# ShigemichiMatsuzaki/MSPL

Hardware: AMD Instinct MI355X
Metric: images/sec pseudo-label gen, ESPDNet-UE s=2.0 480x360(->288x480) bs=16 (higher is better)
Workload: dtype f32; 1 GPU; BASELINE configs[1]: ESPDNet-UE s=2.0 C=13 single-source pseudo-label gen (forward + pred+0.5aux argmax + KL uncertainty + histogram), bs=16/GPU, 16x3x288x480 fp32, hipGraph replay, 3 launches in flight per GPU, 2 consecutive batches of 16 per launch; per_gpu_batch=16, batches_in_flight=3, batches_per_launch=2, classes=13

## Files before the change

### include/mspl_hip.h

```cpp
#ifndef MSPL_HIP_H
#define MSPL_HIP_H

#include <stddef.h>
#include <stdint.h>

#ifdef __cplusplus
extern "C" {
#endif

typedef enum {
    MSPL_OK = 0,
    MSPL_ERR_BAD_SHAPE = -1,
    MSPL_ERR_UNSUPPORTED = -2,
    MSPL_ERR_NULL_POINTER = -3,
    MSPL_ERR_HIP = -4
} mspl_status;

typedef struct {
    const float* scale;
    const float* shift;
    const float* alpha;
    const float* pre_add;
    const float* residual;
    const float* reinf_r;
// ... 46 lines not shown
int mspl_avgpool3x3s2_fwd(const float* x, int32_t N, int32_t C, int32_t H, int32_t W,
                          const mspl_epilogue_t* ep, float* out, void* stream);

int mspl_bilinear_fwd(const float* x, int32_t N, int32_t C, int32_t Hi, int32_t Wi, int32_t Ho,
                      int32_t Wo, int32_t align_corners, const mspl_epilogue_t* ep, float* out, void* stream);

int mspl_decoder_merge_fwd(const float* enc, const float* bu, const float* w3, const float* e_scale, const float* e_shift,
                           const float* e_alpha, const float* gate, const float* b_scale, const float* b_shift,
                           const float* b_alpha, const float* wp, const float* p_scale, const float* p_shift,
                           const float* p_alpha, int32_t N, int32_t Cin, int32_t Cout, int32_t P, int32_t H, int32_t W,
                           float* out, void* stream);

int mspl_adaptive_avgpool_fwd(const float* x, int32_t N, int32_t C, int32_t Hi, int32_t Wi,
                              int32_t Ho, int32_t Wo, const mspl_epilogue_t* ep, float* out,
                              void* stream);

int mspl_pointwise_fwd(const float* x, int32_t N, int32_t C, int32_t HW, const mspl_epilogue_t* ep,
                       float* out, void* stream);

int mspl_gap_gate_fwd(const float* x, const float* w, int32_t N, int32_t Cin, int32_t Cout,
                      int32_t HW, float* mean_ws, float* gate, void* stream);

int mspl_fusion_gate_fwd(const float* z, const float* rgb, const float* depth, int64_t count, float* out, void* stream);
int mspl_fusion_gate_bwd(const float* z, const float* rgb, const float* depth, const float* gy, int64_t count,
                         float* gz, float* grgb, float* gdepth, void* stream);

int mspl_avgpool3x3s2_psum_blocks(int32_t H, int32_t W);
int mspl_avgpool3x3s2_psum_fwd(const float* x, int32_t N, int32_t C, int32_t H, int32_t W, const mspl_epilogue_t* ep, float* out,
                               float* psum, void* stream);
int mspl_gate_from_sums_fwd(const float* psum, const float* w, int32_t N, int32_t Cin, int32_t Cout, int32_t nblk, int32_t HW,
                            float* gate, void* stream);

int mspl_down_head_fits(int32_t N, int32_t nin, int32_t n, int32_t groups, int32_t H, int32_t W, uint32_t launch_flags);
int mspl_down_head_psum_blocks(int32_t H, int32_t W);
int mspl_down_head_fwd(const float* x, const float* wp, const float* pscale, const float* pshift, const float* palpha, int32_t N,
                       int32_t nin, int32_t n, int32_t groups, int32_t H, int32_t W, const mspl_epilogue_t* ep, float* r, float* out,
                       float* psum, void* stream);

int64_t mspl_pyr_down_prep_lds_bytes(int32_t N, int32_t P, int32_t h, int32_t w, int32_t nb, const int32_t* hs,
                                     const int32_t* ws);
int mspl_pyr_down_prep_fwd(const float* x, int32_t N, int32_t P, int32_t h, int32_t w, int32_t nb, const int32_t* hs,
                           const int32_t* ws, const float* const* stage_w, float* const* out, void* stream);
int mspl_pyr_down_prep_train_fwd(const float* x, int32_t N, int32_t P, int32_t h, int32_t w, int32_t nb, const int32_t* hs,
                                 const int32_t* ws, const float* const* stage_w, float* const* out, float* const* pooled,
                                 void* stream);
int mspl_pyr_down_mid_bwd(const float* const* g_e, const float* const* pooled, const float* const* stage_w, int32_t N, int32_t P,
                          int32_t h, int32_t w, int32_t nb, const int32_t* hs, const int32_t* ws, float* const* gw,
                          float* const* gx, void* stream);

int mspl_pyrpool_fused_fwd(const float* x, int32_t N, int32_t P, int32_t h, int32_t w, int32_t nb,
                           const int32_t* hs, const int32_t* ws, const float* const* stage_w,
                           const float* const* down_e, const float* br_scale, const float* br_shift,
                           const float* br_alpha, const float* merge_w, const mspl_epilogue_t* ep,
                           float* out, void* stream);

int mspl_pyrpool_fused_train_fwd(const float* x, int32_t N, int32_t P, int32_t h, int32_t w, int32_t nb,
                                 const int32_t* hs, const int32_t* ws, const float* const* stage_w,
                                 const float* const* down_e, const float* br_scale, const float* br_shift,
                                 const float* br_alpha, const float* merge_w, const mspl_epilogue_t* ep,
                                 float* out, float* zcat, void* stream);
int mspl_pyrpool_fused_train_fits(int32_t N, int32_t P, int32_t h, int32_t w, int32_t nb, const int32_t* hs, const int32_t* ws);
int mspl_pyrpool_merge_bwd(const float* gy, const float* mraw, const float* zcat, int32_t N, int32_t P, int32_t h,
                           int32_t w, int32_t nb, const float* br_scale, const float* br_shift, const float* br_alpha,
                           const float* br_mean, const float* br_inv, const float* merge_w, const float* m_scale,
                           const float* m_shift, const float* m_alpha, const float* m_mean, const float* m_inv,
                           float* gt, float* g_br_scale, float* g_br_shift, float* g_br_alpha, float* g_merge_w,
                           float* g_m_scale, float* g_m_shift, float* g_m_alpha, void* stream);
int mspl_pyrpool_branch_bwd_fits(int32_t N, int32_t P, int32_t h, int32_t w, int32_t nb, const int32_t* hs, const int32_t* ws);
int mspl_pyrpool_branch_bwd(const float* x, int32_t N, int32_t P, int32_t h, int32_t w, int32_t nb, const int32_t* hs,
                            const int32_t* ws, const float* const* stage_w, const float* const* gt, float* const* gw,
                            const float* add0, const float* add1, float* gx, void* stream);

int mspl_label_epilogue_fwd(const float* main, const float* aux, int32_t N, int32_t C,
                            int32_t Hm, int32_t Wm, int32_t Ha, int32_t Wa, int32_t H, int32_t W,
                            const uint8_t* lut, uint8_t* labels, float* prob, float* kld,
                            float* main_up, float* aux_up, void* stream);

int64_t mspl_label_epilogue_hist_workspace_bytes(int32_t N, int32_t H, int32_t W);
int mspl_label_epilogue_hist_fits(int32_t N, int32_t C, int32_t Hm, int32_t Wm, int32_t Ha, int32_t Wa, int32_t H, int32_t W);
int mspl_label_epilogue_hist_fwd(const float* main, const float* aux, int32_t N, int32_t C,
                                 int32_t Hm, int32_t Wm, int32_t Ha, int32_t Wa, int32_t H, int32_t W,
                                 const uint8_t* lut, uint8_t* labels, float* kld, unsigned long long* hist,
                                 int32_t num_classes, void* workspace, int64_t workspace_bytes, void* stream);

int mspl_merge_labels_fwd(const uint8_t* const* src, int32_t S, int64_t npix, int32_t num_classes,
                          int32_t thresh, int32_t fill, uint8_t* out, unsigned long long* hist,
                          void* stream);


int mspl_conv_bwd_data(const float* gy, const float* w, int32_t N, int32_t Cin, int32_t Cout, int32_t groups,
                       int32_t H, int32_t W, int32_t K, int32_t stride, int32_t dilation, int32_t accumulate,
                       float* gx, void* stream);

int mspl_conv_bwd_weight(const float* gy, const float* x, int32_t N, int32_t Cin, int32_t Cout, int32_t groups,
                         int32_t H, int32_t W, int32_t K, int32_t stride, int32_t dilation, int32_t accumulate,
                         float* gw, void* stream);
int mspl_conv1x1_wgrad_batch(const float* const* gy, const float* const* x, float* const* gw, const float* const* rowscale,
                             const int32_t* N, const int32_t* Cin, const int32_t* Cout, const int32_t* groups, const int32_t* HW, int32_t nprob,
                             void* stream);

int mspl_down_tail_fwd(const float* a, const float* b, const float* reinf, const float* alpha, int32_t N, int32_t nin, int32_t C,
                       int32_t HW, float* y, void* stream);
int mspl_down_tail_bwd(const float* a, const float* b, const float* reinf, const float* gy, const float* alpha, int32_t N, int32_t nin,
                       int32_t C, int32_t HW, float* ga, float* gb, float* greinf, float* galpha, void* stream);

int mspl_affine_prelu_bwd(const float* c, const float* pre_add, const float* residual, const float* gy,
                          const float* scale, const float* shift, const float* alpha, int32_t N, int32_t C,
                          int32_t HW, float* gz, float* gc, float* gscale, float* gshift, float* galpha, void* stream);

int mspl_avgpool3x3s2_bwd(const float* gy, int32_t N, int32_t C, int32_t H, int32_t W, float* gx, void* stream);
int mspl_bilinear_bwd(const float* gy, int32_t N, int32_t C, int32_t Hi, int32_t Wi, int32_t Ho, int32_t Wo,
                      float* gx, void* stream);
int mspl_adaptive_avgpool_bwd(const float* gy, int32_t N, int32_t C, int32_t Hi, int32_t Wi, int32_t Ho, int32_t Wo,
                              float* gx, void* stream);

int mspl_plane_dot(const float* a, const float* b, int32_t planes, int32_t HW, float* out, void* stream);
int mspl_plane_broadcast(const float* v, int32_t planes, int32_t HW, float mul, int32_t accumulate, float* gx,
                         void* stream);
int mspl_bn_prelu_bwd(const float* c, const float* pre_add, const float* residual, const float* gy, const float* scale,
                      const float* shift, const float* alpha, const float* bn_mean, const float* bn_inv, int32_t N, int32_t C,
                      int32_t HW, float* gz, float* gc, float* ggamma, float* gbeta, float* galpha, void* stream);
int mspl_gap_gate_bwd(const float* ggate, const float* gate, const float* mean, const float* w, int32_t N,
                      int32_t Cin, int32_t Cout, float* gw, float* gmean, void* stream);
int mspl_gap_gate_bwd_accum(const float* ggate, const float* gate, const float* mean, const float* w, int32_t N,
                      int32_t Cin, int32_t Cout, float* gw, float* gmean, void* stream);
int mspl_hff_suffix_sum(const float* g, int32_t N, int32_t n, int32_t HW, float* out, void* stream);

int mspl_hff_bn_prelu_suffix_bwd(const float* z, const float* gy, const float* scale, const float* shift, const float* alpha,
                                 const float* bn_mean, const float* bn_inv, int32_t N, int32_t n, int32_t HW, float* out,
                                 float* gscale, float* gshift, float* galpha, void* stream);

int mspl_uw_loss_fwd_bwd(const float* pred, const float* aux, const int64_t* target, const float* class_weights,
                         int32_t N, int32_t C, int32_t HW, float ce_scale, float* loss_acc, float* gpred,
                         float* gaux, float* kld_out, void* stream);
int mspl_uw_loss_scaled_fwd_bwd(const float* pred, const float* aux, const int64_t* target, const float* class_weights,
                                int32_t N, int32_t C, int32_t HW, float ce_scale, float out_scale, float* loss_acc,
                                float* gpred, float* gaux, float* kld_out, void* stream);
int mspl_uw_loss_heads_supported(int32_t C);
int mspl_uw_loss_heads_fwd_bwd(const float* main_lo, const float* aux_lo, const int64_t* target, const float* class_weights,
                               int32_t N, int32_t C, int32_t Hm, int32_t Wm, int32_t Ha, int32_t Wa, int32_t H, int32_t W,
                               float ce_scale, float out_scale, float* loss_acc, float* gpred, float* gaux, void* stream);
int mspl_uw_loss_heads_meters_fwd_bwd(const float* main_lo, const float* aux_lo, const int64_t* target, const float* class_weights,
                                      int32_t N, int32_t C, int32_t Hm, int32_t Wm, int32_t Ha, int32_t Wa, int32_t H, int32_t W,
                                      float ce_scale, float out_scale, float* loss_acc, float* gpred, float* gaux,
                                      int32_t miou_classes, float meter_weight, unsigned long long* areas, double* meter, void* stream);

int mspl_dense_conv_fwd(const float* x, const float* w_packed, int32_t N, int32_t Cin, int32_t Cout, int32_t H, int32_t W,
                        int32_t ksize, int32_t dilation, const mspl_epilogue_t* ep, float* out, void* stream);

int mspl_dense_conv_split_fits(int32_t Cin, int32_t Cout, int32_t ksize, int32_t planes);
int mspl_dense_conv_split_fwd(const float* x, const uint16_t* w_split, int32_t N, int32_t Cin, int32_t Cout, int32_t H, int32_t W,
                              int32_t ksize, int32_t dilation, int32_t planes, const mspl_epilogue_t* ep, float* out, void* stream);

int64_t mspl_dense_conv_wgrad_workspace_bytes(int32_t N, int32_t Cin, int32_t Cout, int32_t H, int32_t W, int32_t ksize,
                                              int32_t dilation, int32_t split);
int mspl_dense_conv_wgrad(const float* gy, const float* x, int32_t N, int32_t Cin, int32_t Cout, int32_t H, int32_t W,
                          int32_t ksize, int32_t dilation, int32_t split, void* workspace, int64_t workspace_bytes,
                          float* dw_packed, float* dbias, void* stream);
int mspl_dense_conv_dgrad(const float* const* gy, const float* const* wt_packed, const int32_t* ksize, const int32_t* dilation,
                          int32_t nbranch, int32_t N, int32_t Cg, int32_t Cx, int32_t H, int32_t W, int32_t accumulate,
                          float* gx, void* stream);

int mspl_miou_areas_fwd(const float* logits, const uint8_t* labels, const int64_t* target, int32_t N, int32_t C, int32_t HW,
                        int32_t num_classes, unsigned long long* hist, void* stream);

int mspl_eval_epilogue_fwd(const float* main, const float* aux, const int64_t* target, const float* class_weights,
// ... 139 lines not shown
```

### mspl_amd/_native.py

```python
import ctypes
import os

import torch

_HERE = os.path.dirname(os.path.abspath(__file__))
LIB_PATH = os.environ.get('MSPL_HIP_LIB') or os.path.join(_HERE, 'lib', 'libmspl_hip.so')

c_f32p = ctypes.c_void_p
c_i32 = ctypes.c_int32
c_i64 = ctypes.c_int64


class Epilogue(ctypes.Structure):
    _fields_ = [('scale', ctypes.c_void_p), ('shift', ctypes.c_void_p), ('alpha', ctypes.c_void_p),
                ('pre_add', ctypes.c_void_p), ('residual', ctypes.c_void_p), ('reinf_r', ctypes.c_void_p),
                ('reinf_w', ctypes.c_void_p), ('gate', ctypes.c_void_p),
                ('out_ctot', c_i32), ('out_coff', c_i32), ('raw_out', ctypes.c_void_p),
                ('struct_size', ctypes.c_uint32), ('flags', ctypes.c_uint32)]


class TrainRec(ctypes.Structure):
    _fields_ = [(n, ctypes.c_void_p) for n in ('scale_x', 'scale_y', 'dscale_x', 'dscale_y', 'out_x', 'out_y', 'near_x', 'near_y',
                                               'near_out_x', 'near_out_y')] + \
               [(n, c_i32) for n in ('sh', 'sw', 'pad_h', 'pad_w', 'crop_i', 'crop_j', 'flip', 'reserved')]


FILTER_LANCZOS = 1
FILTER_BILINEAR = 2

ABI_VERSION = 4
ERR_UNSUPPORTED = -2
LAUNCH_THROUGHPUT = 1
LAUNCH_K2_STREAM_OFF = 2
LAUNCH_K2_STREAM_FORCE = 4


_EP = ctypes.POINTER(Epilogue)

SIGNATURES = {
    'mspl_eesp_dw_hff_fwd': [c_f32p, c_f32p, ctypes.POINTER(c_i32), c_i32, c_i32, c_i32, c_i32, c_i32, _EP,
                             c_f32p, ctypes.c_void_p],
    'mspl_eesp_proj_dw_hff_fits': [c_i32] * 6 + [ctypes.POINTER(c_i32), ctypes.c_uint32],
    'mspl_eesp_proj_dw_hff_fwd': [c_f32p] * 6 + [ctypes.POINTER(c_i32)] + [c_i32] * 6 + [_EP, c_f32p, ctypes.c_void_p],
    'mspl_eesp_dw_exp_fits': [c_i32] * 4 + [ctypes.POINTER(c_i32), ctypes.c_uint32],
    'mspl_eesp_dw_exp_pack_floats': [c_i32],
    'mspl_eesp_dw_exp_pack': [c_f32p] * 5 + [c_i32] * 3 + [ctypes.POINTER(c_i32), c_f32p, ctypes.c_void_p],
    'mspl_eesp_dw_exp_fwd': [c_f32p, c_f32p, ctypes.POINTER(c_i32)] + [c_i32] * 4 + [_EP, c_f32p, ctypes.c_void_p],
    'mspl_eesp_dw_exp_next_pack_floats': [c_i32],
    'mspl_eesp_dw_exp_next_pack': [c_f32p, c_i32, c_f32p, ctypes.c_void_p],
    'mspl_eesp_dw_exp_next_fwd': [c_f32p, c_f32p, ctypes.POINTER(c_i32)] + [c_i32] * 4 + [_EP, c_f32p] + [c_f32p] * 5 + [ctypes.c_void_p],
    'mspl_conv1x1_fwd': [c_f32p, c_f32p, c_i32, c_i32, c_i32, c_i32, c_i32, _EP, c_f32p, ctypes.c_void_p],
    'mspl_conv3x3_fwd': [c_f32p, c_f32p, c_i32, c_i32, c_i32, c_i32, c_i32, c_i32, c_i32, c_i32, _EP, c_f32p,
                         ctypes.c_void_p],
    'mspl_avgpool3x3s2_fwd': [c_f32p, c_i32, c_i32, c_i32, c_i32, _EP, c_f32p, ctypes.c_void_p],
    'mspl_bilinear_fwd': [c_f32p, c_i32, c_i32, c_i32, c_i32, c_i32, c_i32, c_i32, _EP, c_f32p, ctypes.c_void_p],
    'mspl_decoder_merge_fwd': [c_f32p] * 14 + [c_i32] * 6 + [c_f32p, ctypes.c_void_p],
    'mspl_adaptive_avgpool_fwd': [c_f32p, c_i32, c_i32, c_i32, c_i32, c_i32, c_i32, _EP, c_f32p, ctypes.c_void_p],
    'mspl_avgpool3x3s2_psum_fwd': [c_f32p, c_i32, c_i32, c_i32, c_i32, _EP, c_f32p, c_f32p, ctypes.c_void_p],
    'mspl_avgpool3x3s2_psum_blocks': [c_i32, c_i32],
    'mspl_down_head_fits': [c_i32] * 6 + [ctypes.c_uint32],
    'mspl_down_head_psum_blocks': [c_i32, c_i32],
    'mspl_down_head_fwd': [c_f32p] * 5 + [c_i32] * 6 + [_EP, c_f32p, c_f32p, c_f32p, ctypes.c_void_p],
    'mspl_gate_from_sums_fwd': [c_f32p, c_f32p, c_i32, c_i32, c_i32, c_i32, c_i32, c_f32p, ctypes.c_void_p],
    'mspl_pointwise_fwd': [c_f32p, c_i32, c_i32, c_i32, _EP, c_f32p, ctypes.c_void_p],
    'mspl_gap_gate_fwd': [c_f32p, c_f32p, c_i32, c_i32, c_i32, c_i32, c_f32p, c_f32p, ctypes.c_void_p],
    'mspl_fusion_gate_fwd': [c_f32p, c_f32p, c_f32p, c_i64, c_f32p, ctypes.c_void_p],
    'mspl_fusion_gate_bwd': [c_f32p, c_f32p, c_f32p, c_f32p, c_i64, c_f32p, c_f32p, c_f32p, ctypes.c_void_p],
    'mspl_pyrpool_fused_fwd': [c_f32p, c_i32, c_i32, c_i32, c_i32, c_i32, ctypes.POINTER(c_i32), ctypes.POINTER(c_i32),
                               ctypes.POINTER(ctypes.c_void_p), ctypes.POINTER(ctypes.c_void_p), c_f32p, c_f32p, c_f32p,
                               c_f32p, _EP, c_f32p, ctypes.c_void_p],
    'mspl_pyrpool_fused_train_fwd': [c_f32p, c_i32, c_i32, c_i32, c_i32, c_i32, ctypes.POINTER(c_i32), ctypes.POINTER(c_i32),
                                     ctypes.POINTER(ctypes.c_void_p), ctypes.POINTER(ctypes.c_void_p), c_f32p, c_f32p, c_f32p,
                                     c_f32p, _EP, c_f32p, c_f32p, ctypes.c_void_p],
    'mspl_pyrpool_fused_train_fits': [c_i32] * 5 + [ctypes.POINTER(c_i32), ctypes.POINTER(c_i32)],
    'mspl_pyrpool_merge_bwd': [c_f32p] * 3 + [c_i32] * 5 + [c_f32p] * 19 + [ctypes.c_void_p],
    'mspl_pyrpool_branch_bwd_fits': [c_i32] * 5 + [ctypes.POINTER(c_i32), ctypes.POINTER(c_i32)],
    'mspl_pyrpool_branch_bwd': [c_f32p] + [c_i32] * 5 + [ctypes.POINTER(c_i32), ctypes.POINTER(c_i32)] +
                               [ctypes.POINTER(ctypes.c_void_p)] * 3 + [c_f32p, c_f32p, c_f32p, ctypes.c_void_p],
    'mspl_label_epilogue_fwd': [c_f32p, c_f32p, c_i32, c_i32, c_i32, c_i32, c_i32, c_i32, c_i32, c_i32,
                                ctypes.c_void_p, ctypes.c_void_p, c_f32p, c_f32p, c_f32p, c_f32p, ctypes.c_void_p],
    'mspl_label_epilogue_hist_fwd': [c_f32p, c_f32p, c_i32, c_i32, c_i32, c_i32, c_i32, c_i32, c_i32, c_i32,
                                     ctypes.c_void_p, ctypes.c_void_p, c_f32p, ctypes.c_void_p, c_i32, ctypes.c_void_p, c_i64,
                                     ctypes.c_void_p],
    'mspl_label_epilogue_hist_workspace_bytes': [c_i32, c_i32, c_i32],
    'mspl_label_epilogue_hist_fits': [c_i32] * 8,
    'mspl_conv_bwd_data': [c_f32p, c_f32p] + [c_i32] * 10 + [c_f32p, ctypes.c_void_p],
    'mspl_conv_bwd_weight': [c_f32p, c_f32p] + [c_i32] * 10 + [c_f32p, ctypes.c_void_p],
    'mspl_affine_prelu_bwd': [c_f32p] * 7 + [c_i32] * 3 + [c_f32p] * 5 + [ctypes.c_void_p],
    'mspl_bn_train_small_fits': [c_i32] * 3,
    'mspl_bn_train_small_fwd': [c_f32p] * 5 + [c_i32] * 3 + [ctypes.c_float] * 2 + [c_f32p] * 2 + [ctypes.c_void_p] + [c_f32p] * 5 + [ctypes.c_void_p],
    'mspl_bn_train_small_bwd': [c_f32p] * 9 + [c_i32] * 4 + [c_f32p] * 5 + [ctypes.c_void_p],
    'mspl_bn_train_prelu_bwd_apply': [c_f32p] * 7 + [c_i32] * 3 + [c_f32p, ctypes.c_void_p],
    'mspl_pyrpool_merge_fwd': [c_f32p] + [c_i32] * 5 + [c_f32p] * 5 + [ctypes.c_void_p],
    'mspl_bn_stats_path_add': [c_f32p] * 4 + [c_i32] * 4 + [ctypes.c_void_p],
    'mspl_bn_fused_workspace_bytes': [c_i32],
    'mspl_bn_batch_stats_fused_fwd': [c_f32p, c_i32, c_i32, c_i32, ctypes.c_float, ctypes.c_float] + [c_f32p] * 4 + [ctypes.c_void_p] + [c_f32p] * 4
                                     + [ctypes.c_void_p, ctypes.c_void_p],
    'mspl_bn_train_prelu_bwd': [c_f32p] * 9 + [c_i32] * 3 + [c_f32p, c_f32p, ctypes.c_void_p, c_i32] + [c_f32p] * 5 + [ctypes.c_void_p],
    'mspl_down_tail_fwd': [c_f32p] * 4 + [c_i32] * 4 + [c_f32p, ctypes.c_void_p],
    'mspl_down_tail_bwd': [c_f32p] * 5 + [c_i32] * 4 + [c_f32p] * 4 + [ctypes.c_void_p],
    'mspl_bn_prelu_bwd': [c_f32p] * 9 + [c_i32] * 3 + [c_f32p] * 5 + [ctypes.c_void_p],
    'mspl_avgpool3x3s2_bwd': [c_f32p, c_i32, c_i32, c_i32, c_i32, c_f32p, ctypes.c_void_p],
    'mspl_bilinear_bwd': [c_f32p] + [c_i32] * 6 + [c_f32p, ctypes.c_void_p],
    'mspl_adaptive_avgpool_bwd': [c_f32p] + [c_i32] * 6 + [c_f32p, ctypes.c_void_p],
    'mspl_plane_dot': [c_f32p, c_f32p, c_i32, c_i32, c_f32p, ctypes.c_void_p],
    'mspl_plane_broadcast': [c_f32p, c_i32, c_i32, ctypes.c_float, c_i32, c_f32p, ctypes.c_void_p],
    'mspl_gap_gate_bwd': [c_f32p] * 4 + [c_i32] * 3 + [c_f32p, c_f32p, ctypes.c_void_p],
    'mspl_gap_gate_bwd_accum': [c_f32p] * 4 + [c_i32] * 3 + [c_f32p, c_f32p, ctypes.c_void_p],
    'mspl_hff_bn_prelu_suffix_bwd': [c_f32p] * 7 + [c_i32] * 3 + [c_f32p] * 4 + [ctypes.c_void_p],
    'mspl_hff_suffix_sum': [c_f32p, c_i32, c_i32, c_i32, c_f32p, ctypes.c_void_p],
    'mspl_uw_loss_fwd_bwd': [c_f32p, c_f32p, ctypes.c_void_p, c_f32p, c_i32, c_i32, c_i32, ctypes.c_float] + [c_f32p] * 4
                            + [ctypes.c_void_p],
    'mspl_uw_loss_scaled_fwd_bwd': [c_f32p, c_f32p, ctypes.c_void_p, c_f32p, c_i32, c_i32, c_i32, ctypes.c_float, ctypes.c_float] + [c_f32p] * 4
                                   + [ctypes.c_void_p],
    'mspl_uw_loss_heads_supported': [c_i32],
    'mspl_uw_loss_heads_fwd_bwd': [c_f32p, c_f32p, ctypes.c_void_p, c_f32p] + [c_i32] * 8 + [ctypes.c_float] * 2 + [c_f32p] * 3 + [ctypes.c_void_p],
    'mspl_uw_loss_heads_meters_fwd_bwd': [c_f32p, c_f32p, ctypes.c_void_p, c_f32p] + [c_i32] * 8 + [ctypes.c_float] * 2 + [c_f32p] * 3 +
                                         [c_i32, ctypes.c_float, ctypes.c_void_p, ctypes.c_void_p, ctypes.c_void_p],
    'mspl_pixelwise_kld_fwd': [c_f32p, c_f32p, c_i32, c_i32, c_i32, c_f32p, ctypes.c_void_p],
    'mspl_pixelwise_kld_bwd': [c_f32p, c_f32p, c_f32p, c_i32, c_i32, c_i32, c_f32p, c_f32p, ctypes.c_void_p],
    'mspl_weighted_ce_fwd': [c_f32p, ctypes.c_void_p, c_f32p, c_f32p, c_i32, c_i32, c_i32, c_i32, c_f32p, ctypes.c_void_p],
    'mspl_weighted_ce_bwd': [c_f32p, ctypes.c_void_p, c_f32p, c_f32p, c_i32, c_i32, c_i32, c_i32, c_f32p, c_f32p, c_f32p, c_f32p,
                             ctypes.c_void_p],
    'mspl_pyr_down_prep_lds_bytes': [c_i32, c_i32, c_i32, c_i32, c_i32, ctypes.POINTER(c_i32), ctypes.POINTER(c_i32)],
    'mspl_pyr_down_prep_fwd': [c_f32p, c_i32, c_i32, c_i32, c_i32, c_i32, ctypes.POINTER(c_i32), ctypes.POINTER(c_i32),
                               ctypes.POINTER(ctypes.c_void_p), ctypes.POINTER(ctypes.c_void_p), ctypes.c_void_p],
    'mspl_pyr_down_prep_train_fwd': [c_f32p, c_i32, c_i32, c_i32, c_i32, c_i32, ctypes.POINTER(c_i32), ctypes.POINTER(c_i32),
                                     ctypes.POINTER(ctypes.c_void_p), ctypes.POINTER(ctypes.c_void_p), ctypes.POINTER(ctypes.c_void_p),
                                     ctypes.c_void_p],
    'mspl_conv1x1_wgrad_batch': [ctypes.POINTER(ctypes.c_void_p)] * 4 + [ctypes.POINTER(c_i32)] * 5 + [c_i32, ctypes.c_void_p],
    'mspl_pyr_down_mid_bwd': [ctypes.POINTER(ctypes.c_void_p)] * 3 + [c_i32] * 5 + [ctypes.POINTER(c_i32)] * 2 +
                             [ctypes.POINTER(ctypes.c_void_p)] * 2 + [ctypes.c_void_p],
    'mspl_dense_conv_fwd': [c_f32p, c_f32p, c_i32, c_i32, c_i32, c_i32, c_i32, c_i32, c_i32, _EP, c_f32p,
                            ctypes.c_void_p],
    'mspl_dense_conv_split_fits': [c_i32] * 4,
    'mspl_dense_conv_split_fwd': [c_f32p, ctypes.c_void_p] + [c_i32] * 8 + [_EP, c_f32p, ctypes.c_void_p],
    'mspl_dense_conv_wgrad_workspace_bytes': [c_i32] * 8,
    'mspl_dense_conv_wgrad': [c_f32p, c_f32p] + [c_i32] * 8 + [ctypes.c_void_p, c_i64, c_f32p, c_f32p, ctypes.c_void_p],
    'mspl_dense_conv_dgrad': [ctypes.POINTER(ctypes.c_void_p)] * 2 + [ctypes.POINTER(c_i32)] * 2 + [c_i32] * 7 + [c_f32p, ctypes.c_void_p],
    'mspl_eval_epilogue_fwd': [c_f32p, c_f32p, ctypes.c_void_p, c_f32p] + [c_i32] * 8 + [ctypes.c_float, c_i32, c_i32, ctypes.c_void_p,
                               ctypes.c_void_p, ctypes.c_void_p, ctypes.c_void_p],
    'mspl_eval_batch_finalize': [ctypes.c_void_p, ctypes.c_void_p, c_i32, ctypes.c_void_p],
    'mspl_ce_meters_fwd': [c_f32p, ctypes.c_void_p, c_f32p, c_i32, c_i32, c_i32, c_i32, c_i32, ctypes.c_void_p, ctypes.c_void_p, ctypes.c_void_p],
    'mspl_ce_flood_finalize': [ctypes.c_void_p, ctypes.c_float, c_i32, c_f32p, ctypes.c_void_p, ctypes.c_void_p],
    'mspl_ce_head_supported': [c_i32],
    'mspl_ce_head_fits': [c_i32] * 6,
    'mspl_ce_head_meters_fwd_bwd': [c_f32p, ctypes.c_void_p, c_f32p] + [c_i32] * 8 + [ctypes.c_void_p, ctypes.c_void_p, c_f32p, ctypes.c_void_p],
    'mspl_miou_areas_fwd': [c_f32p, ctypes.c_void_p, ctypes.c_void_p, c_i32, c_i32, c_i32, c_i32, ctypes.c_void_p, ctypes.c_void_p],
    'mspl_resample_ksize': [c_i32, c_i32],
    'mspl_resample_coeffs': [c_i32, c_i32, ctypes.c_void_p, ctypes.c_void_p],
    'mspl_nearest_index': [c_i32, c_i32, ctypes.c_void_p],
    'mspl_preprocess_u8_fwd': [ctypes.c_void_p] + [c_i32] * 6 + [ctypes.c_void_p, ctypes.c_void_p, c_i32, ctypes.c_void_p,
                               ctypes.c_void_p, c_i32] + [ctypes.c_void_p] * 6,
    'mspl_resize_label_fwd': [ctypes.c_void_p] + [c_i32] * 5 + [ctypes.c_void_p] * 5,
    'mspl_resample_ksize_filter': [c_i32, c_i32, c_i32],
    'mspl_resample_coeffs_filter': [c_i32, c_i32, c_i32, ctypes.c_void_p, ctypes.c_void_p],
    'mspl_train_transform_workspace_bytes': [c_i32] * 4,
    'mspl_train_transform_fwd': [ctypes.c_void_p] * 3 + [c_i32] * 7 + [ctypes.c_void_p] * 5 + [c_i32] * 2 + [ctypes.c_void_p] * 4,
    'mspl_bn_batch_stats_fwd': [c_f32p, c_i32, c_i32, c_i32, ctypes.c_float, ctypes.c_float] + [ctypes.c_void_p] * 6,
    'mspl_sgd_step': [c_f32p, c_f32p, c_f32p, c_i64, ctypes.c_float, ctypes.c_float, ctypes.c_float, c_i32, ctypes.c_void_p],
    'mspl_bn_batch_stats_fold_fwd': [c_f32p, c_i32, c_i32, c_i32, ctypes.c_float, ctypes.c_float] + [c_f32p] * 4 + [ctypes.c_void_p] + [c_f32p] * 4 + [ctypes.c_void_p],
    'mspl_bn_batch_stats_bwd_coeffs': [c_f32p] * 6 + [c_i32, ctypes.c_double, c_i32] + [c_f32p] * 4 + [ctypes.c_void_p],
    'mspl_nid_workspace_floats': [c_i32, c_i32, c_i32, c_i32],
    'mspl_nid_hist_fwd': [c_f32p, c_f32p] + [c_i32] * 5 + [ctypes.c_float, ctypes.c_float, c_f32p, c_f32p, ctypes.c_void_p],
    'mspl_nid_hist_bwd': [c_f32p, c_f32p] + [c_i32] * 5 + [ctypes.c_float, ctypes.c_float, c_f32p, c_f32p, c_f32p, ctypes.c_void_p],
    'mspl_eesp_bwd_fused_fits': [c_i32] * 4 + [ctypes.POINTER(c_i32)],
    'mspl_hff_bn_stat_suffix_bwd': [c_f32p] * 7 + [c_i32] * 3 + [c_f32p, ctypes.c_void_p],
    'mspl_eesp_bwd_fused_bnstat': [c_f32p] * 4 + [ctypes.POINTER(c_i32)] + [c_f32p] * 5 + [c_i32] * 4 + [c_f32p, ctypes.POINTER(ctypes.c_void_p)] + [ctypes.c_void_p],
# ... 65 lines not shown
```

### mspl_amd/csrc/conv1x1.hip

```cpp
#include <stdlib.h>

#include <mutex>

#include "common.hpp"

namespace mspl {

int conv1x1_splitk_try(const float* x, const float* w, int N, int Cin, int Cout, int groups, int HW, const Epi& e, float* out,
                       hipStream_t s);

typedef float floatx16 __attribute__((ext_vector_type(16)));

struct PwGeom {
    int N, Cin, Cout, G, K, M, HW;
    int KS;
    int MB;
    int mblocks;
    int mc_total;
    int WM;
    int TPW;
    int ptiles;
    int pgroups;
    int vecw;
    unsigned long long* stamps;
// ... 649 lines not shown
        }
    }
#pragma unroll
    for (int m = 0; m < MT; ++m) {
        const int ml = mt * MT + m;
        if (ml >= g.M) break;
        const int cabs = e.coff + grp * g.M + ml;
        const EpiCh ec = epi_channel(e, cabs);
        float* dst = out + epi_offset(e, img, cabs, p0);
        if (e.raw) {
            float* rd = e.raw + epi_offset(e, img, cabs, p0);
            if (v4) store_out4(rd, make_float4(acc[m][0], acc[m][1], acc[m][2], acc[m][3]));
            else {
#pragma unroll
                for (int j = 0; j < 4; ++j)
                    if (p0 + j < g.HW) rd[j] = acc[m][j];
            }
        }
        if (v4) {
            store_out4(dst, epi_apply4(e, ec, acc[m], img, cabs, p0));
        } else {
#pragma unroll
            for (int j = 0; j < 4; ++j)
                if (p0 + j < g.HW) dst[j] = epi_apply(e, ec, acc[m][j], img, cabs, p0 + j);
        }
    }
}

template <int MT, int UNR>
__global__ __launch_bounds__(256) void conv1x1_thin_kernel(const float* __restrict__ x, const float* __restrict__ w,
                                                           PwSmall g, Epi e, float* __restrict__ out) {
    extern __shared__ __attribute__((aligned(16))) float wl[];
    const int nw = g.G * g.K * MT;
    for (int i = threadIdx.x; i < nw; i += 256) {
        const int m = i % MT, k = (i / MT) % g.K, grp = i / (MT * g.K);
        wl[i] = m < g.M ? w[((size_t)grp * g.M + m) * g.K + k] : 0.f;
    }
    __syncthreads();
    int slab = blockIdx.z * gridDim.y + blockIdx.y;
    const int q = blockIdx.x * 256 + threadIdx.x;
    if (slab >= g.N * g.G || q >= g.Q) return;
    const int grp = slab % g.G;
    const int img = slab / g.G;
    const int p0 = q * 4;
    const float* xg = x + ((size_t)img * g.Cin + (size_t)grp * g.K) * (size_t)g.HW + p0;
    float acc[MT][4];
#pragma unroll
    for (int m = 0; m < MT; ++m)
#pragma unroll
        for (int j = 0; j < 4; ++j) acc[m][j] = 0.f;
    const float* wk = wl + (size_t)grp * g.K * MT;
    for (int k0 = 0; k0 < g.K; k0 += UNR) {
        float4 xv[UNR];
#pragma unroll
        for (int u = 0; u < UNR; ++u) xv[u] = *reinterpret_cast<const float4*>(xg + (size_t)(k0 + u) * g.HW);
        __builtin_amdgcn_sched_barrier(0);
#pragma unroll
        for (int u = 0; u < UNR; ++u) {
#pragma unroll
            for (int m4 = 0; m4 < MT; m4 += 4) {
                const float4 wv = *reinterpret_cast<const float4*>(wk + (k0 + u) * MT + m4);
                const float ww[4] = {wv.x, wv.y, wv.z, wv.w};
#pragma unroll
                for (int mm = 0; mm < 4; ++mm) {
                    acc[m4 + mm][0] = fmaf(ww[mm], xv[u].x, acc[m4 + mm][0]);
                    acc[m4 + mm][1] = fmaf(ww[mm], xv[u].y, acc[m4 + mm][1]);
                    acc[m4 + mm][2] = fmaf(ww[mm], xv[u].z, acc[m4 + mm][2]);
                    acc[m4 + mm][3] = fmaf(ww[mm], xv[u].w, acc[m4 + mm][3]);
                }
            }
        }
    }
#pragma unroll
    for (int m = 0; m < MT; ++m) {
        if (m < g.M) {
            const int cabs = e.coff + grp * g.M + m;
            const EpiCh ec = epi_channel(e, cabs);
            if (e.raw) store_out4(e.raw + epi_offset(e, img, cabs, p0), make_float4(acc[m][0], acc[m][1], acc[m][2], acc[m][3]));
            store_out4(out + epi_offset(e, img, cabs, p0), epi_apply4(e, ec, acc[m], img, cabs, p0));
        }
    }
}

static int launch_thin_try(const float* x, const float* w, int N, int Cin, int Cout, int groups, int HW, const Epi& e, float* out,
                           hipStream_t s) {
    static const int enabled = MSPL_TUNE_INT("MSPL_PW_THIN", 1);
    const int K = Cin / groups, M = Cout / groups;
    if (!enabled || M > 16 || K < 8 || K > 64 || (K & 7) != 0 || (HW & 3) != 0 ||
        (int64_t)N * groups * ceil_div(HW / 4, 256) < 400)
        return 1;
    if (((uintptr_t)x & 15) || ((uintptr_t)out & 15) || ((uintptr_t)e.raw & 15) || ((uintptr_t)e.pre_add & 15) ||
        ((uintptr_t)e.residual & 15) || ((uintptr_t)e.reinf_r & 15) || ((uintptr_t)e.gate & 15))
        return 1;
    PwSmall g;
    g.N = N; g.Cin = Cin; g.Cout = Cout; g.G = groups; g.K = K; g.M = M; g.HW = HW;
    g.Q = HW / 4;
    g.mtiles = 1;
    const int mt = M <= 8 ? 8 : 16;
    const size_t lds = (size_t)groups * K * mt * sizeof(float);
    if (lds > 48 * 1024) return 1;
    const int64_t slabs = (int64_t)N * groups;
    if (slabs >= 65535ll * 65535ll) return 1;
    const int gy = slabs < 65535 ? (int)slabs : 65535;
    dim3 grid((unsigned)ceil_div(g.Q, 256), (unsigned)gy, (unsigned)ceil_div64(slabs, gy)), blk(256);
    if (mt == 8) hipLaunchKernelGGL((conv1x1_thin_kernel<8, 8>), grid, blk, lds, s, x, w, g, e, out);
    else hipLaunchKernelGGL((conv1x1_thin_kernel<16, 8>), grid, blk, lds, s, x, w, g, e, out);
    return 0;
}

static int launch_pipe(const float* x, const float* w, PwGeom g, const Epi& e, const mspl_epilogue_t* ep, float* out,
                       hipStream_t s) {
    g.KS = g.K | 1;
    int mbr = ((g.M + 31) / 32) * 32;
    if (mbr > 128) mbr = 128;
    static const int dbg_plds = MSPL_TUNE_INT("MSPL_PW_PIPE_LDS", 40);
    while (mbr > 32 && (size_t)mbr * (g.KS + ROWC) * 4 > (size_t)dbg_plds * 1024) mbr -= 32;
    if (mbr == 96) mbr = 64;
    g.MB = mbr;
    g.mblocks = ceil_div(g.M, mbr);
    g.mc_total = mbr / 32;
    g.WM = g.mc_total >= 3 ? 4 : g.mc_total;
    const int wp = 4 / g.WM;
    auto al = [](const void* p, int a) { return p == nullptr || (((uintptr_t)p) & (a - 1)) == 0; };
    auto ok = [&](int ns) {
        const int a = ns * 4;
        return g.HW % ns == 0 && al(x, a) && al(out, a) && (!ep || (al(ep->pre_add, a) && al(ep->residual, a) && al(ep->reinf_r, a)));
    };
    int nsub = ok(2) ? 2 : 1;
    static const int dbg_nsub = MSPL_TUNE_INT("MSPL_PW_NSUB", 0);
    static const int dbg_tpw = MSPL_TUNE_INT("MSPL_PW_TPW", 0);
    if ((dbg_nsub == 1 || dbg_nsub == 2) && ok(dbg_nsub)) nsub = dbg_nsub;
    g.ptiles = (int)ceil_div64((int64_t)g.N * g.HW, 32 * nsub);
    int tpw = 1;
    static const int pipe_wgs = MSPL_TUNE_INT("MSPL_PW_PIPE_WGS", 768);
    while ((int64_t)g.G * g.mblocks * ceil_div(g.ptiles, wp * tpw) > pipe_wgs) ++tpw;
    if (dbg_tpw) tpw = dbg_tpw;
    g.TPW = tpw;
    g.pgroups = ceil_div(g.ptiles, wp * tpw);
    const int64_t blocks = (int64_t)g.G * g.mblocks * g.pgroups;
    MSPL_REQUIRE(blocks < (1ll << 31), MSPL_ERR_BAD_SHAPE, "conv1x1: grid too large");
    const dim3 grid((unsigned)blocks), blk(256);
    {
        static unsigned long long* stamp_buf = nullptr;
        static const int dbg_stamp = MSPL_STAMP_ENV("MSPL_PW_STAMP");
        if (dbg_stamp && !stamp_buf) (void)hipMalloc(&stamp_buf, (size_t)5 * 65536 * sizeof(unsigned long long));
        g.stamps = (dbg_stamp && blocks <= 65536) ? stamp_buf : nullptr;
    }
    g.AR = g.M < g.MB ? g.M : g.MB;
    const size_t lds = ((size_t)g.MB * ROWC + (size_t)g.AR * g.KS) * sizeof(float);
    MSPL_REQUIRE(lds <= 96 * 1024, MSPL_ERR_UNSUPPORTED, "conv1x1: weight tile of %zu B exceeds LDS", lds);
    if (lds > 64 * 1024) {
#define MSPL_PIPE_ATTR(NG) do { (void)hipFuncSetAttribute((const void*)conv1x1_pipe_kernel<2, NG>, hipFuncAttributeMaxDynamicSharedMemorySize, 96 * 1024); \
                                (void)hipFuncSetAttribute((const void*)conv1x1_pipe_kernel<1, NG>, hipFuncAttributeMaxDynamicSharedMemorySize, 96 * 1024); } while (0)
        static std::once_flag attr_once;
        std::call_once(attr_once, [] { MSPL_PIPE_ATTR(8); MSPL_PIPE_ATTR(12); MSPL_PIPE_ATTR(16); (void)hipGetLastError(); });
#undef MSPL_PIPE_ATTR
    }
#define MSPL_PIPE(NG) do { if (nsub == 2) hipLaunchKernelGGL((conv1x1_pipe_kernel<2, NG>), grid, blk, lds, s, x, w, g, e, out); \
                           else hipLaunchKernelGGL((conv1x1_pipe_kernel<1, NG>), grid, blk, lds, s, x, w, g, e, out); } while (0)
    switch (g.K >> 3) {
        case 2: MSPL_PIPE(2); break;
        case 3: MSPL_PIPE(3); break;
        case 4: MSPL_PIPE(4); break;
        case 6: MSPL_PIPE(6); break;
        case 8: MSPL_PIPE(8); break;
        case 12: MSPL_PIPE(12); break;
        case 16: MSPL_PIPE(16); break;
        case 32: MSPL_PIPE(32); break;
        default: MSPL_PIPE(64); break;
    }
#undef MSPL_PIPE
    MSPL_CHECK_LAUNCH("conv1x1(tile-pipelined)");
    if (g.stamps) {
// ... 2 lines not shown
        (void)hipMemcpy(host, g.stamps, (size_t)blocks * 4 * sizeof(unsigned long long), hipMemcpyDeviceToHost);
        unsigned long long t0 = ~0ull, t3 = 0; double a = 0, b = 0, c = 0, late = 0;
        for (int64_t i = 0; i < blocks; ++i) { if (host[4*i] < t0) t0 = host[4*i]; if (host[4*i+3] > t3) t3 = host[4*i+3]; a += host[4*i+1]-host[4*i]; b += host[4*i+2]-host[4*i+1]; c += host[4*i+3]-host[4*i+2]; }
        for (int64_t i = 0; i < blocks; ++i) late += host[4*i] - t0;
        fprintf(stderr, "[pw-pipe stamp] K=%d M=%d HW=%d blocks=%lld tpw=%d span=%.2fus  avg: start-delay=%.2fus fetch+stage+barrier=%.2fus kloop=%.2fus epilogue(+more tiles)=%.2fus\n",
                g.K, g.M, g.HW, (long long)blocks, g.TPW, (t3-t0)/100.0, late/blocks/100.0, a/blocks/100.0, b/blocks/100.0, c/blocks/100.0);
    }
    return MSPL_OK;
}

static int launch_areg(const float* x, const float* w, PwGeom g, const Epi& e, const mspl_epilogue_t* ep, float* out,
                       hipStream_t s) {
    static const int dbg_astage = MSPL_TUNE_INT("MSPL_PW_ASTAGE", -1);
    g.astage = dbg_astage >= 0 ? dbg_astage : !(g.K <= 32 && (int64_t)g.N * g.HW >= 100000);
    g.KS = g.K | 1;
    int mbr = ((g.M + 31) / 32) * 32;
    if (mbr > 128) mbr = 128;
    while (g.astage && mbr > 32 && (size_t)mbr * (g.KS + ROWC) * 4 > 40 * 1024) mbr -= 32;
    if (mbr == 96) mbr = 64;
    g.MB = mbr;
    g.mblocks = ceil_div(g.M, mbr);
    g.mc_total = mbr / 32;
    g.WM = g.mc_total >= 3 ? 4 : g.mc_total;
    const int wp = 4 / g.WM;
    auto al = [](const void* p, int a) { return p == nullptr || (((uintptr_t)p) & (a - 1)) == 0; };
    auto ok = [&](int ns) {
        const int a = ns * 4;
        return g.HW % ns == 0 && al(x, a) && al(out, a) && (!ep || (al(ep->pre_add, a) && al(ep->residual, a) && al(ep->reinf_r, a)));
    };
    auto tiles_of = [&](int ns) { return (int64_t)g.G * g.mblocks * g.mc_total * ceil_div64((int64_t)g.N * g.HW, 32 * ns); };
    int nsub = 1;
    if (ok(2) && tiles_of(2) >= 4096) nsub = 2;
    static const int dbg_nsub = MSPL_TUNE_INT("MSPL_PW_NSUB", 0);
    static const int dbg_tpw = MSPL_TUNE_INT("MSPL_PW_TPW", 0);
    if ((dbg_nsub == 1 || dbg_nsub == 2) && ok(dbg_nsub)) nsub = dbg_nsub;
    g.ptiles = (int)ceil_div64((int64_t)g.N * g.HW, 32 * nsub);
    int tpw = 1;
    while (tpw < 8 && tiles_of(nsub) / (tpw * 2) >= 4096) tpw *= 2;
    if (dbg_tpw) tpw = dbg_tpw;
    g.TPW = tpw;
    g.pgroups = ceil_div(g.ptiles, wp * tpw);
    const int64_t blocks = (int64_t)g.G * g.mblocks * g.pgroups;
    MSPL_REQUIRE(blocks < (1ll << 31), MSPL_ERR_BAD_SHAPE, "conv1x1: grid too large");
    const dim3 grid((unsigned)blocks), blk(256);
    const size_t lds = (size_t)g.MB * (ROWC + (g.astage ? g.KS : 0)) * sizeof(float);
#define MSPL_AREG(NG) do { if (nsub == 2) hipLaunchKernelGGL((conv1x1_areg_kernel<2, NG>), grid, blk, lds, s, x, w, g, e, out); \
                           else hipLaunchKernelGGL((conv1x1_areg_kernel<1, NG>), grid, blk, lds, s, x, w, g, e, out); } while (0)
    switch (g.K >> 3) {
        case 2: MSPL_AREG(2); break;
        case 3: MSPL_AREG(3); break;
        case 4: MSPL_AREG(4); break;
        case 6: MSPL_AREG(6); break;
        case 8: MSPL_AREG(8); break;
        case 12: MSPL_AREG(12); break;
        default: MSPL_AREG(16); break;
    }
#undef MSPL_AREG
    MSPL_CHECK_LAUNCH("conv1x1(register weights)");
    return MSPL_OK;
}

}

using namespace mspl;

static int launch_small(const float* x, const float* w, int N, int Cin, int Cout, int groups, int HW,
                        const Epi& e, float* out, hipStream_t s) {
    PwSmall g;
    g.N = N; g.Cin = Cin; g.Cout = Cout; g.G = groups; g.K = Cin / groups; g.M = Cout / groups; g.HW = HW;
    g.Q = ceil_div(HW, 4);
    const int mt = g.M <= 2 ? 2 : (g.M <= 4 ? 4 : 8);
    g.mtiles = ceil_div(g.M, mt);
    const size_t lds = (size_t)Cout * g.K * sizeof(float);
    MSPL_REQUIRE(lds <= 48 * 1024, MSPL_ERR_UNSUPPORTED, "conv1x1(small-K): weight block %zu B exceeds LDS", lds);
    const int64_t slabs = (int64_t)N * groups * g.mtiles;
    MSPL_REQUIRE(slabs < 65535ll * 65535ll, MSPL_ERR_BAD_SHAPE, "conv1x1: grid too large");
    const int gy = slabs < 65535 ? (int)slabs : 65535;
    dim3 grid((unsigned)ceil_div(g.Q, 256), (unsigned)gy, (unsigned)ceil_div64(slabs, gy)), blk(256);
    if (mt == 2) hipLaunchKernelGGL(conv1x1_valu_kernel<2>, grid, blk, lds, s, x, w, g, e, out);
    else if (mt == 4) hipLaunchKernelGGL(conv1x1_valu_kernel<4>, grid, blk, lds, s, x, w, g, e, out);
    else hipLaunchKernelGGL(conv1x1_valu_kernel<8>, grid, blk, lds, s, x, w, g, e, out);
    MSPL_CHECK_LAUNCH("conv1x1(small-K)");
    return MSPL_OK;
}

extern "C" int mspl_conv1x1_fwd(const float* x, const float* w, int32_t N, int32_t Cin, int32_t Cout,
                                int32_t groups, int32_t HW, const mspl_epilogue_t* ep, float* out,
                                void* stream) {
    MSPL_REQUIRE(x && w && out, MSPL_ERR_NULL_POINTER, "conv1x1: null pointer");
    MSPL_REQUIRE(N > 0 && Cin > 0 && Cout > 0 && groups > 0 && HW > 0, MSPL_ERR_BAD_SHAPE,
                 "conv1x1: bad shape N=%d Cin=%d Cout=%d groups=%d HW=%d", N, Cin, Cout, groups, HW);
    MSPL_REQUIRE(Cin % groups == 0 && Cout % groups == 0, MSPL_ERR_BAD_SHAPE,
                 "conv1x1: channels (%d,%d) not divisible by groups %d", Cin, Cout, groups);
    if (int rc = check_epi(ep, Cout, "conv1x1", true)) return rc;
    const Epi e = make_epi(ep, Cout, HW);
    hipStream_t s = (hipStream_t)stream;
    PwGeom g;
    memset(&g, 0, sizeof(g));
    g.N = N; g.Cin = Cin; g.Cout = Cout; g.G = groups; g.K = Cin / groups; g.M = Cout / groups; g.HW = HW;
    if (launch_thin_try(x, w, N, Cin, Cout, groups, HW, e, out, s) == 0) {
        MSPL_CHECK_LAUNCH("conv1x1(thin)");
        return MSPL_OK;
    }
    if ((g.K < 16 || (g.K & 1)) && (size_t)Cout * g.K * 4 <= 48 * 1024) return launch_small(x, w, N, Cin, Cout, groups, HW, e, out, s);
    MSPL_REQUIRE((g.K & 1) == 0, MSPL_ERR_UNSUPPORTED, "conv1x1: odd K=%d per group with %d output channels is not supported", g.K, Cout);

    if (conv1x1_splitk_try(x, w, N, Cin, Cout, groups, HW, e, out, s) == 0) {
        MSPL_CHECK_LAUNCH("conv1x1(split-K)");
        return MSPL_OK;
    }
    const int K32 = (g.K + 31) & ~31;
    g.KS = K32 | 1;
    g.vecw = ((g.K & 3) == 0) && ((((uintptr_t)w) & 15) == 0);
    static const int dbg_areg = MSPL_TUNE_INT("MSPL_PW_AREG", 1);
    const int ng8 = g.K >> 3;
    const bool ng_ok = ng8 == 2 || ng8 == 3 || ng8 == 4 || ng8 == 6 || ng8 == 8 || ng8 == 12 || ng8 == 16;
    const bool ng_big = (ng8 == 32 || ng8 == 64) && (size_t)((g.M < 32 ? g.M : 32) * ((g.K | 1)) + 32 * ROWC) * 4 <= 64 * 1024 && g.M <= 32;
    const bool areg_shape = dbg_areg == 2 || (g.K <= 32 && (int64_t)N * HW >= 100000);
    static const int dbg_pipe = MSPL_TUNE_INT("MSPL_PW_PIPE", 1);
    const bool pipe_shape = true;
    if (dbg_pipe && pipe_shape && (g.K & 7) == 0 && (ng_ok || ng_big) && g.vecw &&
        (size_t)N * Cin * HW * sizeof(float) < (1ull << 32) && (size_t)N * e.ctot * HW * sizeof(float) < (1ull << 32))
        return launch_pipe(x, w, g, e, ep, out, s);
    if (dbg_areg && areg_shape && (g.K & 7) == 0 && ng_ok && g.vecw &&
        (size_t)N * Cin * HW * sizeof(float) < (1ull << 32) && (size_t)N * e.ctot * HW * sizeof(float) < (1ull << 32))
        return launch_areg(x, w, g, e, ep, out, s);
    const int rowf = ROWC;
    MSPL_REQUIRE((size_t)N * Cin * HW * sizeof(float) < (1ull << 32) && (size_t)N * e.ctot * HW * sizeof(float) < (1ull << 32),
                 MSPL_ERR_UNSUPPORTED, "conv1x1: tensor exceeds the 32-bit byte offsets of the matrix-core kernel");
    const size_t lds_cap = 96 * 1024;
    static const int dbg_lds = MSPL_TUNE_INT("MSPL_PW_LDS", 0);
    const size_t lds_want = dbg_lds ? (size_t)dbg_lds * 1024 : 40 * 1024;
    MSPL_REQUIRE((size_t)32 * (g.KS + rowf) * 4 <= lds_cap, MSPL_ERR_UNSUPPORTED,
                 "conv1x1: K=%d per group exceeds the LDS weight tile", g.K);
    int mb = ((g.M + 31) / 32) * 32;
    if (mb > 128) mb = 128;
    while (mb > 32 && (size_t)mb * (g.KS + rowf) * 4 > lds_want) mb -= 32;
    g.MB = mb;
    g.mblocks = ceil_div(g.M, mb);
    g.mc_total = mb / 32;
    g.WM = g.mc_total >= 3 ? 4 : g.mc_total;
    const int wp = 4 / g.WM;
    const size_t lds = (size_t)g.MB * (g.KS + rowf) * sizeof(float);
    static std::once_flag attr_once;
    {
        constexpr int cap = 96 * 1024;
        std::call_once(attr_once, [] {
            (void)hipFuncSetAttribute((const void*)conv1x1_mfma_kernel<1, 4>, hipFuncAttributeMaxDynamicSharedMemorySize, cap);
            (void)hipFuncSetAttribute((const void*)conv1x1_mfma_kernel<2, 4>, hipFuncAttributeMaxDynamicSharedMemorySize, cap);
            (void)hipFuncSetAttribute((const void*)conv1x1_mfma_kernel<4, 4>, hipFuncAttributeMaxDynamicSharedMemorySize, cap);
            (void)hipFuncSetAttribute((const void*)conv1x1_mfma_kernel<1, 16>, hipFuncAttributeMaxDynamicSharedMemorySize, cap);
            (void)hipFuncSetAttribute((const void*)conv1x1_mfma_kernel<2, 16>, hipFuncAttributeMaxDynamicSharedMemorySize, cap);
            (void)hipFuncSetAttribute((const void*)conv1x1_mfma_kernel<1, 8>, hipFuncAttributeMaxDynamicSharedMemorySize, cap);
            (void)hipFuncSetAttribute((const void*)conv1x1_mfma_kernel<2, 8>, hipFuncAttributeMaxDynamicSharedMemorySize, cap);
            (void)hipGetLastError();
        });
    }
    auto al = [](const void* p, int a) { return p == nullptr || (((uintptr_t)p) & (a - 1)) == 0; };
    auto ok = [&](int ns) {
        const int a = ns * 4;
        return HW % ns == 0 && al(x, a) && al(out, a) && (!ep || (al(ep->pre_add, a) && al(ep->residual, a) && al(ep->reinf_r, a)));
    };
    auto waves_of = [&](int ns) { return (int64_t)groups * g.mblocks * g.mc_total * ceil_div64((int64_t)N * HW, 32 * ns); };
    int nsub = 1;
    if (ok(4) && waves_of(4) >= 2048) nsub = 4;
    else if (ok(2) && waves_of(2) >= 2048) nsub = 2;
// ... 54 lines not shown
```

### mspl_amd/csrc/labels.hip

```cpp
#include <stdlib.h>

#include <algorithm>

#include "common.hpp"
#include "loss_parts.hpp"

namespace mspl {

struct LeGeom {
    int N, C, Hm, Wm, Ha, Wa, H, W;
    float shm, swm, sha, swa;
};

__global__ __launch_bounds__(256) void label_epilogue_kernel(const float* __restrict__ mainp,
                                                             const float* __restrict__ auxp, LeGeom g,
                                                             const uint8_t* __restrict__ lut,
                                                             uint8_t* __restrict__ labels, float* __restrict__ prob,
                                                             float* __restrict__ kld, float* __restrict__ main_up,
                                                             float* __restrict__ aux_up, int64_t total) {
    int64_t idx = (int64_t)blockIdx.x * 256 + threadIdx.x;
    if (idx >= total) return;
    const int x = (int)(idx % g.W);  idx /= g.W;
    const int y = (int)(idx % g.H);
    const int n = (int)(idx / g.H);
// ... 81 lines not shown
    bilinear_src(g.shm, y, g.Hm, my0, my1, mwy0, mwy1);
    bilinear_src(g.swm, x, g.Wm, mx0, mx1, mwx0, mwx1);
    const int mplane = g.Hm * g.Wm;
    const float* mr0 = mainp + (size_t)n * g.C * mplane + my0 * g.Wm;
    const float* mr1 = mainp + (size_t)n * g.C * mplane + my1 * g.Wm;
    float m[CMAX], a[CMAX];
#pragma unroll
    for (int c = 0; c < CMAX; ++c) {
        m[c] = -INFINITY;
        if (c < g.C) {
            const float top = mwx0 * mr0[c * mplane + mx0] + mwx1 * mr0[c * mplane + mx1];
            const float bot = mwx0 * mr1[c * mplane + mx0] + mwx1 * mr1[c * mplane + mx1];
            m[c] = mwy0 * top + mwy1 * bot;
        }
    }
    if (auxp) {
        int ay0, ay1, ax0, ax1;  float awy0, awy1, awx0, awx1;
        bilinear_src(g.sha, y, g.Ha, ay0, ay1, awy0, awy1);
        bilinear_src(g.swa, x, g.Wa, ax0, ax1, awx0, awx1);
        const int aplane = g.Ha * g.Wa;
        const float* ar0 = auxp + (size_t)n * g.C * aplane + ay0 * g.Wa;
        const float* ar1 = auxp + (size_t)n * g.C * aplane + ay1 * g.Wa;
#pragma unroll
        for (int c = 0; c < CMAX; ++c) {
            a[c] = -INFINITY;
            if (c < g.C) {
                const float top = awx0 * ar0[c * aplane + ax0] + awx1 * ar0[c * aplane + ax1];
                const float bot = awx0 * ar1[c * aplane + ax0] + awx1 * ar1[c * aplane + ax1];
                a[c] = awy0 * top + awy1 * bot;
            }
        }
    } else {
#pragma unroll
        for (int c = 0; c < CMAX; ++c) a[c] = c < g.C ? 0.f : -INFINITY;
    }
    const size_t pix = ((size_t)n * g.H + y) * g.W + x;
    if (labels) {
        float omax = -INFINITY;  int best = 0;
#pragma unroll
        for (int c = 0; c < CMAX; ++c) {
            if (c < g.C) { const float o = m[c] + 0.5f * a[c]; if (o > omax) { omax = o; best = c; } }
        }
        labels[pix] = lut ? lut[best] : (uint8_t)best;
    }
    if (kld) {
        float k = 0.f;
        if (auxp) {
            float M1 = -INFINITY, M2 = -INFINITY;
#pragma unroll
            for (int c = 0; c < CMAX; ++c) { M1 = fmaxf(M1, m[c]); M2 = fmaxf(M2, a[c]); }
            float S1 = 0.f, T1 = 0.f, S2 = 0.f;
#pragma unroll
            for (int c = 0; c < CMAX; ++c) {
                if (c < g.C) {
                    const float d1 = m[c] - M1, d2 = a[c] - M2;
                    const float e1 = __expf(d1);
                    S1 += e1;
                    T1 = fmaf(e1, d1 - d2, T1);
                    S2 += __expf(d2);
                }
            }
            k = T1 / S1 - __logf(S1) + __logf(S2);
        }
        kld[pix] = k;
    }
}

constexpr int LE_RB = 4;

struct LeStage {
    int nrm, nra;
    int wms, was;
    int ncls;
    unsigned magc;
    int vec;
    unsigned magqm, magqa;
};

template <int CMAX, bool EXACT, int WMS, int WAS>
__global__ __launch_bounds__(256) void label_epilogue_lds_kernel(const float* __restrict__ mainp, const float* __restrict__ auxp,
                                                                 LeGeom g, LeStage st, const uint8_t* __restrict__ lut,
                                                                 uint8_t* __restrict__ labels, float* __restrict__ kld,
                                                                 unsigned int* __restrict__ hist_ws) {
    extern __shared__ __attribute__((aligned(16))) float smem[];
    float* ml = smem;
    float* al = smem + (size_t)st.nrm * g.C * st.wms;
    unsigned int* sh_hist = reinterpret_cast<unsigned int*>(al + (size_t)st.nra * g.C * st.was);
    const int tid = threadIdx.x;
    const int xb = blockIdx.x * 256;
    const int nbands = (g.H + LE_RB - 1) / LE_RB;
    const int bq = (nbands + 3) >> 2;
    const int band = (int)(blockIdx.y & 3) * bq + (int)(blockIdx.y >> 2), n = blockIdx.z;
    const unsigned blk = (blockIdx.z * gridDim.y + blockIdx.y) * gridDim.x + blockIdx.x;
    if (band >= nbands) {
        if (hist_ws && tid < 32) hist_ws[(size_t)blk * 32 + tid] = 0u;
        return;
    }
    const int y0 = band * LE_RB;
    const int ylast = min(y0 + LE_RB, g.H) - 1, xlast = min(xb + 256, g.W) - 1;
    int rm_lo, rm_hi, cm_lo, cm_hi, t0, t1;  float f0, f1;
    bilinear_src(g.shm, y0, g.Hm, rm_lo, t1, f0, f1);
    bilinear_src(g.shm, ylast, g.Hm, t0, rm_hi, f0, f1);
    bilinear_src(g.swm, xb, g.Wm, cm_lo, t1, f0, f1);
    bilinear_src(g.swm, xlast, g.Wm, t0, cm_hi, f0, f1);
    int ra_lo = 0, ra_hi = -1, ca_lo = 0, ca_hi = -1;
    if (auxp) {
        bilinear_src(g.sha, y0, g.Ha, ra_lo, t1, f0, f1);
        bilinear_src(g.sha, ylast, g.Ha, t0, ra_hi, f0, f1);
        bilinear_src(g.swa, xb, g.Wa, ca_lo, t1, f0, f1);
        bilinear_src(g.swa, xlast, g.Wa, t0, ca_hi, f0, f1);
    }
    if (hist_ws && tid < 32) sh_hist[tid] = 0;

    const int cmA = st.vec ? (cm_lo & ~3) : cm_lo, caA = st.vec ? (ca_lo & ~3) : ca_lo;
    {
        const int mplane = g.Hm * g.Wm, aplane = g.Ha * g.Wa;
        const float* mb = mainp + (size_t)n * g.C * mplane;
        const float* ab = auxp ? auxp + (size_t)n * g.C * aplane : nullptr;
        const int nm = (rm_hi - rm_lo + 1) * g.C, na = auxp ? (ra_hi - ra_lo + 1) * g.C : 0;
        if (st.vec) {
            const int wavei = __builtin_amdgcn_readfirstlane(tid >> 6), lane = tid & 63;
#pragma unroll
            for (int head = 0; head < 2; ++head) {
                const bool ism = head == 0;
                const int cq = ism ? (st.wms >> 2) : (st.was >> 2), npair = ism ? nm : na;
                if (npair == 0) continue;
                const int ppw = cq <= 64 ? 64 / cq : 1;
                const int slot = (int)(((unsigned)lane * (ism ? st.magqm : st.magqa)) >> 20), q = lane - slot * cq;
                const int col = (ism ? cmA : caA) + 4 * q;
                const bool lane_ok = slot < ppw && col < (ism ? g.Wm : g.Wa) && col <= (ism ? cm_hi : ca_hi);
                const float* base = ism ? mb + (size_t)rm_lo * g.Wm + col : ab + (size_t)ra_lo * g.Wa + col;
                const int plane = ism ? mplane : aplane, rowlen = ism ? g.Wm : g.Wa, wst = ism ? st.wms : st.was;
                float* dbase = (ism ? ml : al) + 4 * q;
                constexpr int UL = 4;
                for (int p0 = wavei * ppw + slot; p0 - slot < npair; p0 += 4 * ppw * UL) {
                    float4 v[UL];  int dst[UL];
#pragma unroll
                    for (int u = 0; u < UL; ++u) {
                        const int pair = p0 + u * 4 * ppw;
                        dst[u] = -1;  v[u] = make_float4(0.f, 0.f, 0.f, 0.f);
                        if (lane_ok && pair < npair) {
                            const int row = (int)(((unsigned)pair * st.magc) >> 16), cc = pair - row * g.C;
                            v[u] = *reinterpret_cast<const float4*>(base + (size_t)cc * plane + row * rowlen);
                            dst[u] = pair * wst;
                        }
                    }
                    __builtin_amdgcn_sched_barrier(0);
#pragma unroll
                    for (int u = 0; u < UL; ++u)
                        if (dst[u] >= 0) *reinterpret_cast<float4*>(dbase + dst[u]) = v[u];
                }
            }
        } else {
            const int half = __builtin_amdgcn_readfirstlane(tid >> 7), lane = tid & 127;
            const int wm = cm_hi - cm_lo + 1, wa = ca_hi - ca_lo + 1;
            constexpr int UL = 8;
            for (int base = half; base < nm + na; base += 2 * UL) {
                float v[UL][2];  int dst[UL][2];
#pragma unroll
                for (int u = 0; u < UL; ++u) {
                    const int it = base + 2 * u;
                    dst[u][0] = dst[u][1] = -1;  v[u][0] = v[u][1] = 0.f;
                    if (it < nm + na) {
                        const bool ism = it < nm;
                        const int pair = ism ? it : it - nm;
                        const int row = (int)(((unsigned)pair * st.magc) >> 16), c = pair - row * g.C;
                        const int w = ism ? wm : wa;
                        const float* src = ism ? mb + (size_t)c * mplane + (rm_lo + row) * g.Wm + cm_lo
                                               : ab + (size_t)c * aplane + (ra_lo + row) * g.Wa + ca_lo;
                        const int d0 = ism ? pair * st.wms : (int)(al - ml) + pair * st.was;
#pragma unroll
                        for (int h2 = 0; h2 < 2; ++h2) {
                            const int j = lane + 128 * h2;
                            if (j < w) { v[u][h2] = src[j];  dst[u][h2] = d0 + j; }
                        }
                    }
                }
                __builtin_amdgcn_sched_barrier(0);
#pragma unroll
                for (int u = 0; u < UL; ++u) {
                    if (dst[u][0] >= 0) ml[dst[u][0]] = v[u][0];
                    if (dst[u][1] >= 0) ml[dst[u][1]] = v[u][1];
                }
            }
        }
    }
    __syncthreads();

    const int wms_c = WMS > 0 ? WMS : st.wms, was_c = WAS > 0 ? WAS : st.was;
    const int x = xb + tid;
    unsigned int cnt_mask_lo = 0;
    if (x < g.W) {
#pragma clang fp contract(fast)
        int mx0, mx1, ax0 = 0, ax1 = 0;  float mwx0, mwx1, awx0 = 0.f, awx1 = 0.f;
        bilinear_src(g.swm, x, g.Wm, mx0, mx1, mwx0, mwx1);
        if (auxp) bilinear_src(g.swa, x, g.Wa, ax0, ax1, awx0, awx1);
        const float* mcol = ml + (mx0 - cmA);
        const float* acol = al + (ax0 - caA);
        const int mdx = mx1 - mx0, adx = ax1 - ax0;
        float mtop[CMAX], mbot[CMAX], atop[CMAX], abot[CMAX];
        int mkt = -1, mkb = -1, akt = -1, akb = -1;
#pragma unroll
        for (int c = 0; c < CMAX; ++c) { mtop[c] = mbot[c] = atop[c] = abot[c] = 0.f; }
#pragma unroll 1
        for (int r = 0; r < LE_RB; ++r) {
            const int y = y0 + r;
            unsigned lab8 = 0xffu;
            if (y < g.H) {
                int my0, my1;  float mwy0, mwy1;
                bilinear_src(g.shm, y, g.Hm, my0, my1, mwy0, mwy1);
                if (my0 != mkt) {
                    if (my0 == mkb) {
#pragma unroll
                        for (int c = 0; c < CMAX; ++c) mtop[c] = mbot[c];
                    } else {
                        const float* mr0 = mcol + (my0 - rm_lo) * (EXACT ? CMAX : g.C) * wms_c;
                        const float* mr0b = mr0 + mdx;
#pragma unroll
                        for (int c = 0; c < CMAX; ++c)
                            if (EXACT || c < g.C) mtop[c] = mwx0 * mr0[c * wms_c] + mwx1 * mr0b[c * wms_c];
                    }
                    mkt = my0;
                }
                if (my1 != mkb) {
                    if (my1 == mkt) {
#pragma unroll
                        for (int c = 0; c < CMAX; ++c) mbot[c] = mtop[c];
                    } else {
                        const float* mr1 = mcol + (my1 - rm_lo) * (EXACT ? CMAX : g.C) * wms_c;
                        const float* mr1b = mr1 + mdx;
#pragma unroll
                        for (int c = 0; c < CMAX; ++c)
                            if (EXACT || c < g.C) mbot[c] = mwx0 * mr1[c * wms_c] + mwx1 * mr1b[c * wms_c];
                    }
                    mkb = my1;
                }
                float m[CMAX], a[CMAX];
#pragma unroll
                for (int c = 0; c < CMAX; ++c) m[c] = (EXACT || c < g.C) ? mwy0 * mtop[c] + mwy1 * mbot[c] : -INFINITY;
                if (auxp) {
                    int ay0, ay1;  float awy0, awy1;
                    bilinear_src(g.sha, y, g.Ha, ay0, ay1, awy0, awy1);
                    if (ay0 != akt) {
                        if (ay0 == akb) {
#pragma unroll
                            for (int c = 0; c < CMAX; ++c) atop[c] = abot[c];
                        } else {
                            const float* ar0 = acol + (ay0 - ra_lo) * (EXACT ? CMAX : g.C) * was_c;
                            const float* ar0b = ar0 + adx;
#pragma unroll
                            for (int c = 0; c < CMAX; ++c)
                                if (EXACT || c < g.C) atop[c] = awx0 * ar0[c * was_c] + awx1 * ar0b[c * was_c];
                        }
                        akt = ay0;
                    }
                    if (ay1 != akb) {
                        if (ay1 == akt) {
#pragma unroll
                            for (int c = 0; c < CMAX; ++c) abot[c] = atop[c];
                        } else {
                            const float* ar1 = acol + (ay1 - ra_lo) * (EXACT ? CMAX : g.C) * was_c;
                            const float* ar1b = ar1 + adx;
#pragma unroll
                            for (int c = 0; c < CMAX; ++c)
                                if (EXACT || c < g.C) abot[c] = awx0 * ar1[c * was_c] + awx1 * ar1b[c * was_c];
                        }
                        akb = ay1;
                    }
#pragma unroll
                    for (int c = 0; c < CMAX; ++c) a[c] = (EXACT || c < g.C) ? awy0 * atop[c] + awy1 * abot[c] : -INFINITY;
                } else {
#pragma unroll
                    for (int c = 0; c < CMAX; ++c) a[c] = (EXACT || c < g.C) ? 0.f : -INFINITY;
                }
                const size_t pix = ((size_t)n * g.H + y) * g.W + x;
                if (labels) {
                    float omax = -INFINITY;  int best = 0;
#pragma unroll
                    for (int c = 0; c < CMAX; ++c) {
                        if (EXACT || c < g.C) { const float o = m[c] + 0.5f * a[c]; if (o > omax) { omax = o; best = c; } }
                    }
                    lab8 = lut ? (unsigned)lut[best] : (unsigned)best;
                    labels[pix] = (uint8_t)lab8;
                }
                if (kld) {
                    float k = 0.f;
                    if (auxp) {
                        float M1 = -INFINITY, M2 = -INFINITY;
#pragma unroll
                        for (int c = 0; c < CMAX; ++c) { M1 = fmaxf(M1, m[c]); M2 = fmaxf(M2, a[c]); }
                        float S1 = 0.f, T1 = 0.f, S2 = 0.f;
#pragma unroll
                        for (int c = 0; c < CMAX; ++c) {
                            if (EXACT || c < g.C) {
                                const float d1 = m[c] - M1, d2 = a[c] - M2;
                                const float e1 = __expf(d1);
                                S1 += e1;
                                T1 = fmaf(e1, d1 - d2, T1);
                                S2 += __expf(d2);
                            }
                        }
                        k = T1 / S1 - __logf(S1) + __logf(S2);
                    }
                    kld[pix] = k;
                }
            }
            cnt_mask_lo |= lab8 << (8 * r);
        }
    } else {
        cnt_mask_lo = 0xffffffffu;
    }
    if (hist_ws) {
        for (int c = 0; c < st.ncls; ++c) {
            unsigned cnt = 0;
#pragma unroll
            for (int r = 0; r < LE_RB; ++r)
                cnt += (unsigned)__builtin_popcountll(__builtin_amdgcn_ballot_w64(((cnt_mask_lo >> (8 * r)) & 0xffu) == (unsigned)c));
            if ((tid & 63) == 0 && cnt) atomicAdd(&sh_hist[c], cnt);
        }
        __syncthreads();
        if (tid < 32) hist_ws[(size_t)blk * 32 + tid] = tid < st.ncls ? sh_hist[tid] : 0u;
    }
}

constexpr int LE_RED = 16;
__global__ __launch_bounds__(256) void label_hist_reduce_kernel(const unsigned int* __restrict__ ws, int nrows, int ncls,
                                                                unsigned long long* __restrict__ hist) {
    __shared__ unsigned int part[8][32];
    const int c = threadIdx.x & 31, sub = threadIdx.x >> 5;
    unsigned int s = 0;
    const int step = 8 * LE_RED;
    int r = blockIdx.x * 8 + sub;
    for (; r + 7 * step < nrows; r += 8 * step) {
        unsigned int v[8];
#pragma unroll
        for (int u = 0; u < 8; ++u) v[u] = ws[(size_t)(r + u * step) * 32 + c];
#pragma unroll
        for (int u = 0; u < 8; ++u) s += v[u];
    }
    for (; r < nrows; r += step) s += ws[(size_t)r * 32 + c];
    part[sub][c] = s;
    __syncthreads();
    if (threadIdx.x < 32 && (int)threadIdx.x < ncls) {
        unsigned long long t = 0;
#pragma unroll
        for (int i = 0; i < 8; ++i) t += part[i][threadIdx.x];
        if (t) atomicAdd(&hist[threadIdx.x], t);
    }
}

struct MergeSrc {
    const uint8_t* p[8];
};

template <int S, int NCLS>
__global__ __launch_bounds__(256) void merge_labels_kernel(MergeSrc src, int64_t npix, int ncls, int thresh,
                                                           int fill, uint8_t* __restrict__ out,
                                                           unsigned long long* __restrict__ hist, int vec_ok) {
    uint32_t h[NCLS];
#pragma unroll
    for (int c = 0; c < NCLS; ++c) h[c] = 0;
    const int64_t nchunks = (npix + 15) >> 4;
    for (int64_t ch = (int64_t)blockIdx.x * 256 + threadIdx.x; ch < nchunks; ch += (int64_t)gridDim.x * 256) {
        const int64_t p0 = ch << 4;
        const int cnt = (int)((npix - p0) < 16 ? (npix - p0) : 16);
        uint32_t words[S][4];
        if (vec_ok && cnt == 16) {
#pragma unroll
            for (int s = 0; s < S; ++s) {
                const uint4 v = *reinterpret_cast<const uint4*>(src.p[s] + p0);
                words[s][0] = v.x; words[s][1] = v.y; words[s][2] = v.z; words[s][3] = v.w;
            }
        } else {
#pragma unroll
            for (int s = 0; s < S; ++s) {
#pragma unroll
                for (int q = 0; q < 4; ++q) {
                    uint32_t wv = 0;
                    for (int b = 0; b < 4; ++b) {
                        const int i = q * 4 + b;
                        if (i < cnt) wv |= (uint32_t)src.p[s][p0 + i] << (8 * b);
                    }
                    words[s][q] = wv;
                }
            }
        }
        uint32_t res[4];
#pragma unroll
        for (int q = 0; q < 4; ++q) {
            uint32_t r = 0;
#pragma unroll
            for (int b = 0; b < 4; ++b) {
                uint32_t lab[S];
#pragma unroll
                for (int s = 0; s < S; ++s) lab[s] = (words[s][q] >> (8 * b)) & 0xFFu;
                int best = 0, bestc = -1;
#pragma unroll
                for (int c = 0; c < NCLS; ++c) {
                    if (c < ncls) {
                        int cn = 0;
#pragma unroll
                        for (int s = 0; s < S; ++s) cn += (lab[s] == (uint32_t)c);
                        if (cn > bestc) { bestc = cn; best = c; }
                    }
                }
// ... 121 lines not shown
#define MSPL_LE_ATTR(CM, EX, A, B) ok = hipFuncSetAttribute((const void*)label_epilogue_lds_kernel<CM, EX, A, B>, hipFuncAttributeMaxDynamicSharedMemorySize, 128 * 1024) == hipSuccess && ok
                MSPL_LE_ATTR(5, true, 0, 0);  MSPL_LE_ATTR(5, true, 132, 68);
                MSPL_LE_ATTR(13, true, 0, 0); MSPL_LE_ATTR(13, true, 132, 68);
                MSPL_LE_ATTR(20, true, 0, 0); MSPL_LE_ATTR(20, true, 132, 68);
                MSPL_LE_ATTR(8, false, 0, 0); MSPL_LE_ATTR(16, false, 0, 0); MSPL_LE_ATTR(24, false, 0, 0);
#undef MSPL_LE_ATTR
                (void)hipGetLastError();
                return ok;
            }();
            MSPL_REQUIRE(big_lds || lds <= 64 * 1024, MSPL_ERR_HIP, "label_epilogue: could not raise the dynamic LDS limit");
#define MSPL_LE_LAUNCH(CM, EX) do { if (wide480) hipLaunchKernelGGL((label_epilogue_lds_kernel<CM, EX, 132, 68>), grid, dim3(256), lds, st_, mainp, aux, g, st, lut, labels, kld, ws); \
                                   else hipLaunchKernelGGL((label_epilogue_lds_kernel<CM, EX, 0, 0>), grid, dim3(256), lds, st_, mainp, aux, g, st, lut, labels, kld, ws); } while (0)
            const bool wide480 = (C == 5 || C == 13 || C == 20) && st.wms == 132 && (!aux || st.was == 68);
            if (C == 5) MSPL_LE_LAUNCH(5, true);
            else if (C == 13) MSPL_LE_LAUNCH(13, true);
            else if (C == 20) MSPL_LE_LAUNCH(20, true);
            else if (C <= 8) { if (wide480) return MSPL_ERR_UNSUPPORTED; hipLaunchKernelGGL((label_epilogue_lds_kernel<8, false, 0, 0>), grid, dim3(256), lds, st_, mainp, aux, g, st, lut, labels, kld, ws); }
            else if (C <= 16) hipLaunchKernelGGL((label_epilogue_lds_kernel<16, false, 0, 0>), grid, dim3(256), lds, st_, mainp, aux, g, st, lut, labels, kld, ws);
            else hipLaunchKernelGGL((label_epilogue_lds_kernel<24, false, 0, 0>), grid, dim3(256), lds, st_, mainp, aux, g, st, lut, labels, kld, ws);
#undef MSPL_LE_LAUNCH
            MSPL_CHECK_LAUNCH("label_epilogue");
            if (hist) {
                hipLaunchKernelGGL(label_hist_reduce_kernel, dim3(LE_RED), dim3(256), 0, st_, ws, (int)le_blocks(N, H, W), ncls, hist);
                MSPL_CHECK_LAUNCH("label_epilogue(histogram)");
            }
            return MSPL_OK;
        }
        MSPL_REQUIRE(!hist, MSPL_ERR_UNSUPPORTED, "label_epilogue_hist: tile does not fit the LDS-staged form (N=%d C=%d %dx%d -> %dx%d)",
                     N, C, Hm, Wm, H, W);
        const dim3 grid((unsigned)ceil_div(W, 256), (unsigned)(4 * ceil_div(H, 4)), (unsigned)N);
        MSPL_REQUIRE(H <= 65535, MSPL_ERR_BAD_SHAPE, "label_epilogue: %d rows", H);
        if (C <= 8) hipLaunchKernelGGL(label_epilogue_reg_kernel<8>, grid, dim3(256), 0, st_, mainp, aux, g, lut, labels, kld);
        else if (C <= 16) hipLaunchKernelGGL(label_epilogue_reg_kernel<16>, grid, dim3(256), 0, st_, mainp, aux, g, lut, labels, kld);
        else hipLaunchKernelGGL(label_epilogue_reg_kernel<24>, grid, dim3(256), 0, st_, mainp, aux, g, lut, labels, kld);
        MSPL_CHECK_LAUNCH("label_epilogue");
        return MSPL_OK;
    }
    MSPL_REQUIRE(!hist, MSPL_ERR_UNSUPPORTED, "label_epilogue_hist: shape outside the label-pass form (N=%d C=%d H=%d)", N, C, H);
    hipLaunchKernelGGL(label_epilogue_kernel, dim3((unsigned)ceil_div64(total, 256)), dim3(256), 0, st_,
                       mainp, aux, g, lut, labels, prob, kld, main_up, aux_up, total);
    MSPL_CHECK_LAUNCH("label_epilogue");
    return MSPL_OK;
}

extern "C" int mspl_label_epilogue_fwd(const float* mainp, const float* aux, int32_t N, int32_t C,
                                       int32_t Hm, int32_t Wm, int32_t Ha, int32_t Wa, int32_t H, int32_t W,
                                       const uint8_t* lut, uint8_t* labels, float* prob, float* kld,
                                       float* main_up, float* aux_up, void* stream) {
    return label_epilogue_impl(mainp, aux, N, C, Hm, Wm, Ha, Wa, H, W, lut, labels, prob, kld, main_up, aux_up, nullptr, 0, nullptr, 0,
                               stream);
}

extern "C" int64_t mspl_label_epilogue_hist_workspace_bytes(int32_t N, int32_t H, int32_t W) {
    if (N <= 0 || H <= 0 || W <= 0) return 0;
    return le_blocks(N, H, W) * 32 * (int64_t)sizeof(unsigned int);
}

extern "C" int mspl_label_epilogue_hist_fits(int32_t N, int32_t C, int32_t Hm, int32_t Wm, int32_t Ha, int32_t Wa, int32_t H, int32_t W) {
    if (N <= 0 || C <= 0 || C > 24 || Hm <= 0 || Wm <= 0 || H <= 0 || W <= 0 || Ha < 0 || Wa < 0) return 0;
    const bool aux = Ha > 0 && Wa > 0;
    if (!(H <= 65535 * LE_RB / 4 && N <= 65535 && (int64_t)N * C * Hm * Wm < (1ll << 31) && (int64_t)N * C * (int64_t)Ha * Wa < (1ll << 31))) return 0;
    const bool vec = (Wm % 4 == 0) && (!aux || Wa % 4 == 0);
    const int nrm = bilinear_span(Hm, H, LE_RB, false), nra = aux ? bilinear_span(Ha, H, LE_RB, false) : 0;
    int wms = bilinear_span(Wm, W, 256, vec), was = aux ? bilinear_span(Wa, W, 256, vec) : 4;
    if (!vec) { wms = (wms + 3) & ~3; was = (was + 3) & ~3; }
    const int wms4 = (bilinear_span(Wm, W, 256, true) + 3) & ~3, was4 = aux ? (bilinear_span(Wa, W, 256, true) + 3) & ~3 : 4;
    wms = std::max(wms, wms4); was = std::max(was, was4);
    const size_t lds = ((size_t)nrm * C * wms + (size_t)nra * C * was + 32) * sizeof(float);
    return lds <= 128 * 1024 && (nrm + nra) * C < 4096 && wms <= 256 && was <= 256;
}

extern "C" int mspl_label_epilogue_hist_fwd(const float* mainp, const float* aux, int32_t N, int32_t C,
                                            int32_t Hm, int32_t Wm, int32_t Ha, int32_t Wa, int32_t H, int32_t W,
                                            const uint8_t* lut, uint8_t* labels, float* kld, unsigned long long* hist,
                                            int32_t num_classes, void* workspace, int64_t workspace_bytes, void* stream) {
    MSPL_REQUIRE(labels && hist, MSPL_ERR_NULL_POINTER, "label_epilogue_hist: labels and hist are required");
    MSPL_REQUIRE(num_classes >= 1 && num_classes <= 32, MSPL_ERR_UNSUPPORTED, "label_epilogue_hist: %d classes (1..32)", num_classes);
    MSPL_REQUIRE(C <= 24, MSPL_ERR_UNSUPPORTED, "label_epilogue_hist: %d logit channels (the fused form holds <= 24 in registers; "
                 "use label_epilogue + merge_labels)", C);
    return label_epilogue_impl(mainp, aux, N, C, Hm, Wm, Ha, Wa, H, W, lut, labels, nullptr, kld, nullptr, nullptr, hist, num_classes,
                               workspace, workspace_bytes, stream);
}

extern "C" int mspl_merge_labels_fwd(const uint8_t* const* src, int32_t S, int64_t npix, int32_t num_classes,
                                     int32_t thresh, int32_t fill, uint8_t* out, unsigned long long* hist,
                                     void* stream) {
    MSPL_REQUIRE(src && out, MSPL_ERR_NULL_POINTER, "merge_labels: null pointer");
    MSPL_REQUIRE(S >= 1 && S <= 8, MSPL_ERR_UNSUPPORTED, "merge_labels: %d sources (1..8)", S);
    MSPL_REQUIRE(num_classes >= 1 && num_classes <= 32, MSPL_ERR_UNSUPPORTED, "merge_labels: %d classes (1..32)", num_classes);
    MSPL_REQUIRE(fill >= 0 && fill <= 255, MSPL_ERR_BAD_SHAPE, "merge_labels: fill %d", fill);
    MSPL_REQUIRE(npix >= 0, MSPL_ERR_BAD_SHAPE, "merge_labels: negative pixel count");
    if (npix == 0) return MSPL_OK;
    MergeSrc ms;
    int vec_ok = (((uintptr_t)out) & 15) == 0;
    for (int s = 0; s < 8; ++s) {
        ms.p[s] = s < S ? src[s] : nullptr;
        if (s < S) {
            MSPL_REQUIRE(src[s], MSPL_ERR_NULL_POINTER, "merge_labels: source %d is null", s);
            vec_ok = vec_ok && ((((uintptr_t)src[s]) & 15) == 0);
        }
    }
    const int64_t nchunks = (npix + 15) >> 4;
    int64_t blocks = ceil_div64(nchunks, 256);
    if (blocks > 16384) blocks = 16384;
    dim3 grid((unsigned)blocks);
    hipStream_t st = (hipStream_t)stream;
    switch (S) {
        case 1: launch_merge<1>(num_classes, grid, st, ms, npix, thresh, fill, out, hist, vec_ok); break;
        case 2: launch_merge<2>(num_classes, grid, st, ms, npix, thresh, fill, out, hist, vec_ok); break;
        case 3: launch_merge<3>(num_classes, grid, st, ms, npix, thresh, fill, out, hist, vec_ok); break;
        case 4: launch_merge<4>(num_classes, grid, st, ms, npix, thresh, fill, out, hist, vec_ok); break;
        case 5: launch_merge<5>(num_classes, grid, st, ms, npix, thresh, fill, out, hist, vec_ok); break;
        case 6: launch_merge<6>(num_classes, grid, st, ms, npix, thresh, fill, out, hist, vec_ok); break;
        case 7: launch_merge<7>(num_classes, grid, st, ms, npix, thresh, fill, out, hist, vec_ok); break;
        default: launch_merge<8>(num_classes, grid, st, ms, npix, thresh, fill, out, hist, vec_ok); break;
    }
    MSPL_CHECK_LAUNCH("merge_labels");
    return MSPL_OK;
}

extern "C" int mspl_miou_areas_fwd(const float* logits, const uint8_t* labels, const int64_t* target, int32_t N, int32_t C,
                                   int32_t HW, int32_t num_classes, unsigned long long* hist, void* stream) {
    MSPL_REQUIRE((logits != nullptr) != (labels != nullptr), MSPL_ERR_NULL_POINTER, "miou_areas: pass logits OR labels");
    MSPL_REQUIRE(target && hist, MSPL_ERR_NULL_POINTER, "miou_areas: null pointer");
    MSPL_REQUIRE(N > 0 && HW > 0 && (!logits || C > 0), MSPL_ERR_BAD_SHAPE, "miou_areas: bad shape N=%d C=%d HW=%d", N, C, HW);
    MSPL_REQUIRE(num_classes >= 1 && num_classes <= 64, MSPL_ERR_UNSUPPORTED, "miou_areas: %d classes (1..64)", num_classes);
    const int64_t total = (int64_t)N * HW;
    int64_t blocks = ceil_div64(total, 256 * 8);
    if (blocks > 4096) blocks = 4096;
    if (blocks < 1) blocks = 1;
    hipLaunchKernelGGL(miou_areas_kernel, dim3((unsigned)blocks), dim3(256), 0, (hipStream_t)stream, logits, labels, target, C, HW,
                       num_classes, total, hist);
    MSPL_CHECK_LAUNCH("miou_areas");
    return MSPL_OK;
}
```

### mspl_amd/layers.py

```python
import math
import os
import weakref

import torch
from torch import nn

from . import autograd as ag
from . import ops
from .ops import Epi

config_inp_reinf = 3
PYR_SCALES = (2.0, 1.5, 1.0, 0.5, 0.1)


_PARAM_EPOCH = [0]


def bump_param_epoch():
    _PARAM_EPOCH[0] += 1


def _key(tensors):
    return (_PARAM_EPOCH[0],) + tuple((t.data_ptr(), t._version) for t in tensors)


def cached(module, name, deps, builder):
    store = module.__dict__.setdefault('_mspl_cache', {})
    k = _key(deps)
    hit = store.get(name)
    if hit is None or hit[0] != k:
        with torch.no_grad():
            val = builder()
        store[name] = hit = (k, val)
    return hit[1]


def _require_eval(bn):
    if bn.training:
        raise RuntimeError('mspl_amd: BatchNorm in training mode under torch.no_grad(): the fused inference kernels fold the '
                           'running statistics; call model.eval() (the uest label pass runs frozen BN, '
                           'uest_seg_multi_os.py:605-608), or enable gradients for the batch-statistics training path')


def bn_fold(bn):
    _require_eval(bn)

    def build():
        scale = bn.weight * torch.rsqrt(bn.running_var + bn.eps)
        return scale.contiguous(), (bn.bias - bn.running_mean * scale).contiguous()
    return cached(bn, 'fold', [bn.weight, bn.bias, bn.running_mean, bn.running_var], build)


_SIDE_ENABLED = os.environ.get('MSPL_SIDE_STREAMS', '1') != '0'
_SIDE_STREAMS = {}


class side_streams(object):

    def __init__(self, enabled):
        self.enabled = enabled

    def __enter__(self):
        global _SIDE_ENABLED
        self.prev = _SIDE_ENABLED
        _SIDE_ENABLED = self.enabled and os.environ.get('MSPL_SIDE_STREAMS', '1') != '0'

    def __exit__(self, *exc):
        global _SIDE_ENABLED
        _SIDE_ENABLED = self.prev


def _side_stream(idx, device, parent):
    dev = device.index if device.index is not None else torch.cuda.current_device()
    key = (dev, idx, parent.cuda_stream)
    st = _SIDE_STREAMS.get(key)
    if st is None:
        st = _SIDE_STREAMS[key] = torch.cuda.Stream(device=dev)
    return st


class fork(object):

    def __init__(self, idx, inputs=()):
        self.idx, self.inputs, self.ctx = idx, inputs, None

    def __enter__(self):
        if not _SIDE_ENABLED or _training_path() or not self.inputs:
            return self
        cur = torch.cuda.current_stream(self.inputs[0].device)
        side = _side_stream(self.idx, self.inputs[0].device, cur)
        side.wait_stream(cur)
        for t in self.inputs:
            t.record_stream(side)
        self.ctx = torch.cuda.stream(side)
        self.ctx.__enter__()
        return self

    def __exit__(self, *exc):
        if self.ctx is not None:
            self.ctx.__exit__(*exc)
        return False

    def mark(self):
        if self.ctx is None:
            return None
        ev = torch.cuda.Event()
        ev.record(torch.cuda.current_stream())
        return ev


def wait_mark(ev, outputs=()):
    if ev is None:
        return
    cur = torch.cuda.current_stream()
    cur.wait_event(ev)
    for t in outputs:
        if t is not None:
            t.record_stream(cur)


def join(idx, outputs=()):
    outs = [t for t in outputs if t is not None]
    if not _SIDE_ENABLED or _training_path() or not outs:
        return
    cur = torch.cuda.current_stream(outs[0].device)
    cur.wait_stream(_side_stream(idx, outs[0].device, cur))
    for t in outs:
        t.record_stream(cur)


def _training_path():
    return torch.is_grad_enabled()


def _conv_train(x, conv):
    if conv.kernel_size[0] == 3 and conv.dilation[0] != 1:
        raise RuntimeError('mspl_amd: dilated 3x3 convolutions only occur inside EESP (fused branch op)')
    return ag.conv(x, conv.weight, conv.stride[0], conv.groups)


def _bn_act(z, bn, alpha=None, pre_add=None, residual=None):
    if bn.training:
        if pre_add is not None:
            z, pre_add = z + pre_add, None
        if _FUSED_BN_TRAIN:
            return ag.bn_train_prelu(z, bn, alpha, residual)
        scale, shift = ag.bn_batch_stats(z, bn)
    else:
        scale, shift = train_fold(bn)
        return ag.bn_prelu(z, bn, scale, shift, alpha, pre_add=pre_add, residual=residual)
    return ag.affine_prelu(z, scale, shift, alpha, pre_add=pre_add, residual=residual)

# ... 470 lines not shown
                h = ops.bilinear(x, (h_s, w_s))
                h = ops.conv3x3(h, stage.weight, P)
                ops.adaptive_avgpool(h, (height, width), ep, out=dst)
            else:
                ops.conv3x3(x, stage.weight, P, ep=ep, out=dst)
        mcbr = self.merge_layer[2]
        return ops.conv3x3(cat, mcbr.cbr[0].weight, P, 1, shuffle_groups=S, ep=mcbr.epi())

    def forward_fused(self, x, sizes):
        N, P, height, width = x.shape
        stage_ws, down_es = [], []
        down = [i for i, (h_s, w_s) in enumerate(sizes) if self.scales[i] < 1.0 and (h_s, w_s) != (height, width)]
        prepped = {}
        if down and ops.pyr_down_prep_fits(x.shape, [sizes[i] for i in down]):
            maps = ops.pyr_down_prep(x, [sizes[i] for i in down], [self.stages[i].weight for i in down])
            prepped = dict(zip(down, maps))
        for i, (stage, (h_s, w_s)) in enumerate(zip(self.stages, sizes)):
            if i in down:
                stage_ws.append(None)
                down_es.append(prepped[i] if i in prepped else
                               ops.conv3x3(ops.adaptive_avgpool(x, (h_s, w_s)), stage.weight, P))
            else:
                stage_ws.append(stage.weight)
                down_es.append(None)
        br = self.merge_layer[0].br
        bscale, bshift = bn_fold(br[0])
        mcbr = self.merge_layer[2]
        return ops.pyrpool_fused(x, sizes, stage_ws, down_es, bscale, bshift, br[1].weight, mcbr.cbr[0].weight,
                                 mcbr.epi())

    def _body_train_fused(self, x, sizes):
        bn0, act0 = self.merge_layer[0].br[0], self.merge_layer[0].br[1]
        mcbr = self.merge_layer[2].cbr
        conv2, bn2, act2 = mcbr[0], mcbr[1], mcbr[2]
        folds = [ag.frozen_bn_fold(bn, *train_fold(bn)) for bn in (bn0, bn2)]
        return ag.PyrBodyFn.apply(x, sizes, *folds, bn0.weight, bn0.bias, act0.weight, conv2.weight, bn2.weight,
                                  bn2.bias, act2.weight, *[st.weight for st in self.stages])

    def _body_train_bn(self, x, sizes):
        bn0, act0 = self.merge_layer[0].br[0], self.merge_layer[0].br[1]
        mcbr = self.merge_layer[2].cbr
        conv2, bn2, act2 = mcbr[0], mcbr[1], mcbr[2]
        return ag.PyrBodyBNFn.apply(x, sizes, ag.bn_train_params(bn0, x.device), ag.bn_train_params(bn2, x.device), bn0.weight, bn0.bias,
                                    act0.weight, conv2.weight, bn2.weight, bn2.bias, act2.weight, *[st.weight for st in self.stages])

    def _forward_train(self, x):
        x = self.projection_layer(x)
        height, width = x.shape[2:]
        P = self.proj_planes
        sizes = self.branch_sizes(height, width)
        bn0, bn2 = self.merge_layer[0].br[0], self.merge_layer[2].cbr[1]
        frozen = not (bn0.training or bn2.training)
        both_train = bn0.training and bn2.training
        if _FUSED_PYR_TRAIN and (frozen or both_train) and ag.pyr_body_fits(x.shape, sizes) and (frozen or (height * width) % 4 == 0):
            out = self._body_train_fused(x, sizes) if frozen else self._body_train_bn(x, sizes)
            conv = self.merge_layer[3]
            if self.last_layer_br:
                return _conv_bn_act(out, conv, self.br.br[0], self.br.br[1].weight)
            return ag.conv_affine_prelu(out, conv.weight, 1, 1, None, conv.bias, None)
        hs = []
        xs = ag.fan_out(x, len(self.stages))
        for xb, stage, sc, (h_s, w_s) in zip(xs, self.stages, self.scales, self.branch_sizes(height, width)):
            if sc < 1.0:
                h = ag.adaptive_avgpool(xb, (h_s, w_s))
                h = ag.conv(h, stage.weight, 1, P)
                h = ag.bilinear(h, (height, width))
            elif sc > 1.0:
                h = ag.bilinear(xb, (h_s, w_s))
                h = ag.conv(h, stage.weight, 1, P)
                h = ag.adaptive_avgpool(h, (height, width))
            else:
                h = ag.conv(xb, stage.weight, 1, P)
            hs.append(h)
        out = self.merge_layer[0](torch.cat(hs, 1))
        out = self.merge_layer[1](out)
        out = self.merge_layer[2](out)
        conv = self.merge_layer[3]
        if self.last_layer_br:
            return _conv_bn_act(out, conv, self.br.br[0], self.br.br[1].weight)
        if _FUSED_TRAIN_FWD:
            return ag.conv_affine_prelu(out, conv.weight, 1, 1, None, conv.bias, None)
        return ag.affine_prelu(ag.conv(out, conv.weight, 1, 1), None, conv.bias, None)

    def forward(self, x, fused=True, projected=False):
        if _training_path():
            return self._forward_train(x)
        if not projected:
            x = self.projection_layer(x)
        height, width = x.shape[2:]
        sizes = self.branch_sizes(height, width)
        ok = fused and self._fusable(sizes, height, width) and all(
            (s >= 1.0) or (hs <= height and ws <= width) for s, (hs, ws) in zip(self.scales, sizes))
        m = self.forward_fused(x, sizes) if ok else self.forward_unfused(x)
        return ops.conv1x1(m, self.merge_layer[3].weight, 1, self._final_epilogue())


class EfficientPWConv(nn.Module):
    def __init__(self, nin, nout):
        super().__init__()
        self.wt_layer = nn.Sequential(
            nn.AdaptiveAvgPool2d(output_size=1),
            nn.Conv2d(nin, nout, kernel_size=1, stride=1, padding=0, groups=1, bias=False),
            nn.Sigmoid())
        self.groups = math.gcd(nin, nout)
        self.expansion_layer = DecCBR(nin, nout, kSize=3, stride=1, groups=self.groups)
        self.out_size = nout
        self.in_size = nin

    def forward(self, x, _alias=None):
        if _training_path():
            gate = ag.gap_gate(x, self.wt_layer[1].weight)
            return ag.channel_scale(self.expansion_layer(x if _alias is None else _alias), gate)
        return self.expand(x, self.gate(x))

    def gate(self, x):
        sums = _recall_plane_sums(x)
        if sums is not None:
            return ops.gate_from_sums(sums, self.wt_layer[1].weight, x.shape[2] * x.shape[3])
        return ops.gap_gate(x, self.wt_layer[1].weight)

    def expand(self, x, gate):
        return ops.conv3x3(x, self.expansion_layer.cbr[0].weight, self.groups, ep=self.expansion_layer.epi(gate=gate))

    def __repr__(self):
        return '%s(in_channels=%d, out_channels=%d)' % (self.__class__.__name__, self.in_size, self.out_size)


def decoder_stage_fusable(merge, enc, pyr):
    return (_FUSED_DEC_MERGE and not _training_path() and
            ops.decoder_merge_shape_ok(merge.in_size, merge.out_size, pyr.proj_planes, enc.shape[2], enc.shape[3]))


def decoder_stage_fused(merge, enc, gate, bu_lowres, br_seq, pyr):
    if tuple(enc.shape[2:]) != (bu_lowres.shape[2] * 2, bu_lowres.shape[3] * 2):
        raise RuntimeError('The size of tensor a (%d) must match the size of tensor b (%d) at non-singleton dimension 2'
                           % (enc.shape[2], bu_lowres.shape[2] * 2))
    exp, proj = merge.expansion_layer.cbr, pyr.projection_layer.cbr
    return ops.decoder_merge(enc, bu_lowres, exp[0].weight, tuple(bn_fold(exp[1])) + (exp[2].weight,), gate,
                             tuple(bn_fold(br_seq[0])) + (br_seq[1].weight,), proj[0].weight, tuple(bn_fold(proj[1])) + (proj[2].weight,))


def decoder_merge(pw_out, bu_lowres, br_seq):
    size = (bu_lowres.shape[2] * 2, bu_lowres.shape[3] * 2)
    if tuple(pw_out.shape[2:]) != size:
        raise RuntimeError('The size of tensor a (%d) must match the size of tensor b (%d) at non-singleton dimension 2'
                           % (pw_out.shape[2], size[0]))
    if _training_path():
        return _bn_act(ag.bilinear(bu_lowres, size), br_seq[0], br_seq[1].weight, pre_add=pw_out)
    scale, shift = bn_fold(br_seq[0])
    return ops.bilinear(bu_lowres, size, Epi(scale, shift, br_seq[1].weight, pre_add=pw_out))
```

### mspl_amd/models.py

```python
import copy
import os

import torch
from torch import nn
from torch.nn import init

from . import ops
from . import autograd as ag
from .layers import (C, CBR, DownSampler, EESP, EfficientPWConv, EfficientPyrPool, ImagePyramid, _training_path, cached, run_eesp_chain,
                     decoder_stage_fusable, decoder_stage_fused,
                     decoder_merge, fork, join, wait_mark)

sc_ch_dict = {
    0.5: [16, 32, 64, 128, 256, 1024],
    1.0: [32, 64, 128, 256, 512, 1024],
    1.25: [32, 80, 160, 320, 640, 1024],
    1.5: [32, 96, 192, 384, 768, 1024],
    2.0: [32, 128, 256, 512, 1024, 1280],
}
rep_layers = [0, 3, 7, 3]
recept_limit = [13, 11, 9, 7, 5]
branches = 4
input_reinforcement = True

# ... 80 lines not shown
        w_rgb, w_d = cached(self, 'halves', [w], lambda: (w[:, :c].contiguous(), w[:, c:].contiguous()))
        z = ops.conv1x1(rgb, w_rgb)
        z = ops.conv1x1(depth, w_d, ep=ops.Epi(pre_add=z))
        return ops.fusion_gate(z, rgb, depth)


class _SegBase(nn.Module):
    def _build_decoder(self, config, classes, dataset, pyr_plane_proj, with_aux, aux_layer=2):
        base = DEC_FEAT[dataset]
        dec = [4 * base, 3 * base, 2 * base, classes]
        self.bu_dec_l1 = EfficientPyrPool(in_planes=config[3], proj_planes=pyr_plane_proj, out_planes=dec[0])
        self.bu_dec_l2 = EfficientPyrPool(in_planes=dec[0], proj_planes=pyr_plane_proj, out_planes=dec[1])
        self.bu_dec_l3 = EfficientPyrPool(in_planes=dec[1], proj_planes=pyr_plane_proj, out_planes=dec[2])
        self.bu_dec_l4 = EfficientPyrPool(in_planes=dec[2], proj_planes=pyr_plane_proj, out_planes=dec[3],
                                          last_layer_br=False)
        self.merge_enc_dec_l2 = EfficientPWConv(config[2], dec[0])
        self.merge_enc_dec_l3 = EfficientPWConv(config[1], dec[1])
        self.merge_enc_dec_l4 = EfficientPWConv(config[0], dec[2])
        self.bu_br_l2 = nn.Sequential(nn.BatchNorm2d(dec[0]), nn.PReLU(dec[0]))
        self.bu_br_l3 = nn.Sequential(nn.BatchNorm2d(dec[1]), nn.PReLU(dec[1]))
        self.bu_br_l4 = nn.Sequential(nn.BatchNorm2d(dec[2]), nn.PReLU(dec[2]))
        if with_aux:
            self.aux_layer = aux_layer
            if 0 <= aux_layer < 3:
                self.aux_decoder = EfficientPyrPool(in_planes=dec[aux_layer], proj_planes=pyr_plane_proj,
                                                    out_planes=dec[3], last_layer_br=False)

    def _encode(self, x, image_for_l2, l3_tail, pyr=None):
        b = self.base_net
        if not b.input_reinforcement:
            pyr = None
        elif pyr is None:
            pyr = ImagePyramid(x.detach())
        l1 = b.level1(x)
        if _training_path():
            a1 = ag.fan_out(l1, 4)
            l2 = b.level2_0(a1[0], pyr if image_for_l2 else None, _alias=a1[1])
            a2 = ag.fan_out(l2, 4)
            l3 = b.level3_0(a2[0], pyr, _alias=a2[1])
            for i, layer in enumerate(b.level3):
                l3 = (layer if i == 0 else l3_tail[i])(l3)
            a3 = ag.fan_out(l3, 4)
            l4 = b.level4_0(a3[0], pyr, _alias=a3[1])
            for layer in b.level4:
                l4 = layer(l4)
            return a1[2:], a2[2:], a3[2:], l4
        l2 = b.level2_0(l1, pyr if image_for_l2 else None)
        l3 = b.level3_0(l2, pyr)
        l3 = run_eesp_chain([layer if i == 0 else l3_tail[i] for i, layer in enumerate(b.level3)], l3)
        l4 = b.level4_0(l3, pyr)
        l4 = run_eesp_chain(b.level4, l4)
        return l1, l2, l3, l4

    def _encode_rgbd(self, x, x_d):
        if x_d.dim() != 4 or x_d.shape[0] != x.shape[0] or x_d.shape[1] != 1 or x_d.shape[2:] != x.shape[2:]:
            raise RuntimeError('mspl_amd: depth input %s does not match image %s (expected (N,1,H,W))'
                               % (tuple(x_d.shape), tuple(x.shape)))
        b, d = self.base_net, self.depth_base_net
        pyr = ImagePyramid(x.detach()) if b.input_reinforcement else None
        dl1 = d.level1(x_d)
        l1 = self.fusion_gate_level1(b.level1(x), dl1)
        dl2 = d.level2_0(dl1)
        l2 = self.fusion_gate_level2(b.level2_0(l1, pyr), dl2)
        l3 = b.level3_0(l2, pyr)
        dl3 = d.level3_0(dl2)
        for i, (layer, dlayer) in enumerate(zip(b.level3, d.level3)):
            l3 = (layer if i == 0 else dlayer)(l3)
            dl3 = dlayer(dl3)
            if self.dense_fuse:
                l3 = self.fusion_gate_level3(l3, dl3)
        if not self.dense_fuse:
            l3 = self.fusion_gate_level3(l3, dl3)
        l4 = b.level4_0(l3, pyr)
        dl4 = d.level4_0(dl3)
        for layer, dlayer in zip(b.level4, d.level4):
            l4 = layer(l4)
            dl4 = dlayer(dl4)
            if self.dense_fuse:
                l4 = self.fusion_gate_level4(l4, dl4)
        if not self.dense_fuse:
            l4 = self.fusion_gate_level4(l4, dl4)
        return l1, l2, l3, l4

    def _decode(self, l1, l2, l3, l4, aux_layer):
        aux = None
        st2 = (self.merge_enc_dec_l2, self.bu_br_l2, self.bu_dec_l2)
        st3 = (self.merge_enc_dec_l3, self.bu_br_l3, self.bu_dec_l3)
        st4 = (self.merge_enc_dec_l4, self.bu_br_l4, self.bu_dec_l4)
        if isinstance(l1, tuple):
            pw2 = self.merge_enc_dec_l2(l3[0], _alias=l3[1])
            pw3 = self.merge_enc_dec_l3(l2[0], _alias=l2[1])
            pw4 = self.merge_enc_dec_l4(l1[0], _alias=l1[1])
            e2 = e3 = e4 = None
            l1, l2, l3 = l1[0], l2[0], l3[0]
        else:
          def skip(st, enc):
              return st[0].gate(enc) if decoder_stage_fusable(st[0], enc, st[2]) else st[0](enc)
          with fork(1, (l1, l2, l3)) as f:
            pw2 = skip(st2, l3);  e2 = f.mark()
            pw3 = skip(st3, l2);  e3 = f.mark()
            pw4 = skip(st4, l1);  e4 = f.mark()
        bu = self.bu_dec_l1(l4)
        if aux_layer == 0:
            with fork(2, (bu,)):
                aux = self.aux_decoder(bu)
        wait_mark(e2, (pw2,))
        bu = self._decode_stage(st2, l3, pw2, bu)
        if aux_layer == 1:
            with fork(2, (bu,)):
                aux = self.aux_decoder(bu)
        wait_mark(e3, (pw3,))
        bu = self._decode_stage(st3, l2, pw3, bu)
        if aux_layer == 2:
            with fork(2, (bu,)):
                aux = self.aux_decoder(bu)
        wait_mark(e4, (pw4,))
        bu = self._decode_stage(st4, l1, pw4, bu)
        join(2, (aux,))
        return bu, aux

    @staticmethod
    def _decode_stage(st, enc, pw, bu):
        merge, br, pyr = st
        if pw.dim() == 2:
            proj = decoder_stage_fused(merge, enc, pw, bu, br, pyr)
            if proj is not None:
                return pyr(proj, projected=True)
            pw = merge.expand(enc, pw)
        return pyr(decoder_merge(pw, bu, br))

    def get_basenet_params(self):
        return _param_gen([self.base_net])

    def get_segment_params(self):
        return _param_gen([self.bu_dec_l1, self.bu_dec_l2, self.bu_dec_l3, self.bu_dec_l4, self.merge_enc_dec_l4,
                           self.merge_enc_dec_l3, self.merge_enc_dec_l2, self.bu_br_l4, self.bu_br_l3, self.bu_br_l2])

    def upsample(self, x):
        return ops.bilinear(x, (x.shape[2] * 2, x.shape[3] * 2))


def _check_input(x):
    if x.dim() != 4:
        raise RuntimeError('mspl_amd: expected an (N,C,H,W) batch, got %s' % (tuple(x.shape),))
    if x.shape[2] % 16 or x.shape[3] % 16:
        raise RuntimeError('The size of tensor a must match the size of tensor b: input %dx%d is not a multiple of 16 '
                           '(mspl_amd: H/W not multiple of 16)' % (x.shape[2], x.shape[3]))


class ESPDNetwithUncertaintyEstimation(_SegBase):
    def __init__(self, args, classes=21, dataset='pascal', dense_fuse=False, trainable_fusion=True, aux_layer=2,
                 fix_pyr_plane_proj=False):
        super().__init__()
        self.base_net = EESPNet(args)
        config = self.base_net.config
        tmp_args = copy.deepcopy(args)
        tmp_args.channels = 1
        self.depth_base_net = EESPNet(tmp_args)
        self.fusion_gate_level1 = FusionGate(nchannel=32, is_trainable=trainable_fusion)
        self.fusion_gate_level2 = FusionGate(nchannel=128, is_trainable=trainable_fusion)
        self.fusion_gate_level3 = FusionGate(nchannel=256, is_trainable=trainable_fusion)
        self.fusion_gate_level4 = FusionGate(nchannel=512, is_trainable=trainable_fusion)
        base = DEC_FEAT[dataset]
        pyr = base if fix_pyr_plane_proj else min(classes // 2, base)
        self._build_decoder(config, classes, dataset, pyr, True, aux_layer)
        _init_params(self)
        self.dense_fuse = dense_fuse
        self.classes = classes

    def get_depth_encoder_params(self):
        return _param_gen([self.depth_base_net])

    def get_classification_layer_params(self):
        return self.get_segment_params()

    def forward_lowres(self, x, x_d=None, pyr=None):
        _check_input(x)
        if x_d is None:
            l1, l2, l3, l4 = self._encode(x, True, self.depth_base_net.level3, pyr)
            return self._decode(l1, l2, l3, l4, self.aux_layer)
        l1, l2, l3, l4 = self._encode_rgbd(x, x_d)
        return self._decode(l1, l2, l3, l4, self.aux_layer)

    def forward(self, x, x_d=None):
        main, aux = self.forward_lowres(x, x_d)
        if _training_path():
            return ag.bilinear(main, tuple(x.shape[2:])), ag.bilinear(aux, tuple(x.shape[2:]))
        r = ops.label_epilogue(main, aux, x.shape[2:], want_labels=False, want_logits=True)
        return r['main_up'], r['aux_up']


class ESPDNetSegmentation(_SegBase):

    def __init__(self, args, classes=21, dataset='pascal', dense_fuse=False, trainable_fusion=True):
        super().__init__()
        if dataset == 'forest':
            raise KeyError('forest')
        self.base_net = EESPNet(args)
        config = self.base_net.config
        tmp_args = copy.deepcopy(args)
        tmp_args.channels = 1
        self.depth_base_net = EESPNet(tmp_args)
        self.fusion_gate_level1 = FusionGate(nchannel=32, is_trainable=trainable_fusion)
        self.fusion_gate_level2 = FusionGate(nchannel=128, is_trainable=trainable_fusion)
        self.fusion_gate_level3 = FusionGate(nchannel=256, is_trainable=trainable_fusion)
        self.fusion_gate_level4 = FusionGate(nchannel=512, is_trainable=trainable_fusion)
        self._build_decoder(config, classes, dataset, min(classes // 2, DEC_FEAT[dataset]), False)
        _init_params(self)
        self.dense_fuse = dense_fuse
        self.classes = classes

    def get_depth_encoder_params(self):
        return _param_gen([self.depth_base_net])

    def forward_lowres(self, x, x_d=None):
        _check_input(x)
        if x_d is None:
            l1, l2, l3, l4 = self._encode(x, True, self.depth_base_net.level3)
        else:
            l1, l2, l3, l4 = self._encode_rgbd(x, x_d)
        return self._decode(l1, l2, l3, l4, -1)[0], None

    def forward(self, x, x_d=None):
        main, _ = self.forward_lowres(x, x_d)
        if _training_path():
            return ag.bilinear(main, tuple(x.shape[2:]))
        return ops.bilinear(main, x.shape[2:])


class ESPNetv2Segmentation(_SegBase):
    def __init__(self, args, classes=21, dataset='pascal'):
        super().__init__()
        self.base_net = EESPNet(args)
        config = self.base_net.config
        self._build_decoder(config, classes, dataset, min(classes // 2, DEC_FEAT[dataset]), False)
        _init_params(self)
        self.classes = classes

    def forward_lowres(self, x):
        _check_input(x)
        l1, l2, l3, l4 = self._encode(x, False, self.base_net.level3)
        return self._decode(l1, l2, l3, l4, -1)[0], None

    def forward(self, x):
        main, _ = self.forward_lowres(x)
        if _training_path():
            return ag.bilinear(main, tuple(x.shape[2:]))
        return ops.bilinear(main, x.shape[2:])


def _load_file(weights):
    if not os.path.isfile(weights):
        raise FileNotFoundError('Weight file does not exist at {}. Please check.'.format(weights))
    return torch.load(weights, map_location='cpu')


def espdnetue_seg2(args, load_entire_weights=False, fix_pyr_plane_proj=False):
    model = ESPDNetwithUncertaintyEstimation(args, classes=args.classes, dataset=args.dataset,
                                             dense_fuse=args.dense_fuse, trainable_fusion=args.trainable_fusion,
                                             fix_pyr_plane_proj=fix_pyr_plane_proj)
    weights = args.weights
    if weights:
        pretrained = _load_file(weights)
        model_dict = model.state_dict()
        if load_entire_weights:
            overlap = {k: v for k, v in pretrained.items() if k in model_dict and model_dict[k].size() == v.size()}
            if len(overlap) == 0:
                raise RuntimeError('No overlaping weights between model file and pretrained weight file. Please check')
            model_dict.update(overlap)
            model.load_state_dict(model_dict)
        else:
            base_dict = model.base_net.state_dict()
            overlap = {k.replace('base_net.', ''): v for k, v in pretrained.items()
                       if k.replace('base_net.', '') in base_dict}
            if len(overlap) == 0:
                raise RuntimeError('No overlaping weights between model file and pretrained weight file. Please check')
            base_dict.update(overlap)
            model.base_net.load_state_dict(base_dict)
        d_dict = model.depth_base_net.state_dict()
        overlap = {k.lstrip('base_net.'): v for k, v in pretrained.items() if k.lstrip('base_net.') in d_dict}
        if 'level1.conv.weight' in overlap:
            overlap['level1.conv.weight'] = torch.mean(overlap['level1.conv.weight'], dim=1, keepdim=True)
        if len(overlap) == 0:
            raise RuntimeError('No overlaping weights between model file and pretrained weight file. Please check')
        d_dict.update(overlap)
        model.depth_base_net.load_state_dict(d_dict)
    return model


def espdnetue_seg(args, load_entire_weights=False):
    model = ESPDNetwithUncertaintyEstimation(args, classes=args.classes, dataset=args.dataset,
                                             dense_fuse=args.dense_fuse, trainable_fusion=args.trainable_fusion)
    weights = args.weights
    if weights:
        pretrained = _load_file(weights)
        if load_entire_weights:
            model_dict = model.state_dict()
            overlap = {k: v for k, v in pretrained.items() if k in model_dict}
            if len(overlap) == 0:
                raise RuntimeError('No overlaping weights between model file and pretrained weight file. Please check')
            model_dict.update(overlap)
            model.load_state_dict(model_dict)
        else:
            base_dict = model.base_net.state_dict()
            overlap = {k.replace('base_net.', ''): v for k, v in pretrained.items()
                       if k.replace('base_net.', '') in base_dict}
            if len(overlap) == 0:
                raise RuntimeError('No overlaping weights between model file and pretrained weight file. Please check')
            base_dict.update(overlap)
            model.base_net.load_state_dict(base_dict)
        d_dict = model.depth_base_net.state_dict()
        overlap = {k.lstrip('base_net.'): v for k, v in pretrained.items() if k.lstrip('base_net.') in d_dict}
        overlap['level1.conv.weight'] = torch.mean(overlap['level1.conv.weight'], dim=1, keepdim=True)
        d_dict.update(overlap)
        model.depth_base_net.load_state_dict(d_dict)
    return model


def espnetv2_seg(args):
    model = ESPNetv2Segmentation(args, classes=args.classes, dataset=args.dataset)
    if args.weights:
        pretrained = _load_file(args.weights)
        base_dict = model.base_net.state_dict()
        overlap = {k: v for k, v in pretrained.items() if k in base_dict}
        if len(overlap) == 0:
# ... 39 lines not shown
```

### mspl_amd/ops.py

```python
import ctypes
import math

import torch

from . import _native as nat
from ._native import Epilogue, check, lib


def _stream():
    return ctypes.c_void_p(torch.cuda.current_stream().cuda_stream)


def _f32(t, name):
    if not isinstance(t, torch.Tensor) or not t.is_cuda:
        raise RuntimeError('mspl_amd: %s must be a CUDA (ROCm) tensor; there is no CPU path' % name)
    if t.dtype != torch.float32:
        raise RuntimeError('mspl_amd: %s must be float32, got %s' % (name, t.dtype))
    if not t.is_contiguous():
        t = t.contiguous()
    return t


def _p(t):
    return None if t is None else ctypes.c_void_p(t.data_ptr())
# ... 513 lines not shown
    for i in range(nb):
        if stage_ws[i] is not None:
            t = _f32(stage_ws[i], 'stage weight')
            if t.numel() != P * 9:
                raise RuntimeError('mspl_amd: pyrpool stage weight %s, expected (%d,1,3,3)' % (tuple(t.shape), P))
            keep.append(t)
            sw[i] = t.data_ptr()
        if down_es[i] is not None:
            t = _f32(down_es[i], 'down map')
            if tuple(t.shape) != (N, P, int(sizes[i][0]), int(sizes[i][1])):
                raise RuntimeError('mspl_amd: pyrpool low-res map %s does not match branch size %s' % (tuple(t.shape), sizes[i]))
            keep.append(t)
            de[i] = t.data_ptr()
    bs, bh, ba = _vec(br_scale, nb * P, 'br_scale'), _vec(br_shift, nb * P, 'br_shift'), _vec(br_alpha, nb * P, 'br_alpha')
    dst, coff = _dest(out, (N, P, h, w), x)
    s, k2 = _build(ep, dst, coff, N, P, h * w)
    check(lib.mspl_pyrpool_fused_fwd(_p(x), N, P, h, w, nb, hs, ws, sw, de, _p(bs), _p(bh), _p(ba), _p(merge_w),
                                     ctypes.byref(s), _p(dst), _stream()))
    return dst


def label_epilogue(main, aux, size, lut=None, want_labels=True, want_prob=False, want_kld=False,
                   want_logits=False):
    main = _f32(main, 'main')
    N, C, Hm, Wm = main.shape
    Ha = Wa = 0
    if aux is not None:
        aux = _f32(aux, 'aux')
        if aux.shape[0] != N or aux.shape[1] != C:
            raise RuntimeError('mspl_amd: aux logits %s do not match main %s' % (tuple(aux.shape), tuple(main.shape)))
        Ha, Wa = aux.shape[2:]
    H, W = int(size[0]), int(size[1])
    dev = main.device
    res = {}
    if lut is not None:
        if lut.dtype != torch.uint8 or not lut.is_cuda or lut.numel() < C:
            raise RuntimeError('mspl_amd: lut must be a CUDA uint8 tensor with >= %d entries' % C)
    if want_labels:
        res['labels'] = torch.empty((N, H, W), device=dev, dtype=torch.uint8)
    if want_prob:
        res['prob'] = torch.empty((N, C, H, W), device=dev, dtype=torch.float32)
    if want_kld:
        res['kld'] = torch.empty((N, H, W), device=dev, dtype=torch.float32)
    if want_logits:
        res['main_up'] = torch.empty((N, C, H, W), device=dev, dtype=torch.float32)
        if aux is not None:
            res['aux_up'] = torch.empty((N, C, H, W), device=dev, dtype=torch.float32)
    check(lib.mspl_label_epilogue_fwd(_p(main), _p(aux), N, C, Hm, Wm, Ha, Wa, H, W, _p(lut), _p(res.get('labels')),
                                      _p(res.get('prob')), _p(res.get('kld')), _p(res.get('main_up')),
                                      _p(res.get('aux_up')), _stream()))
    return res


def label_epilogue_hist_fits(main, aux, size):
    N, C, Hm, Wm = [int(v) for v in main.shape]
    Ha, Wa = ([int(v) for v in aux.shape[2:]] if aux is not None else (0, 0))
    return bool(lib.mspl_label_epilogue_hist_fits(N, C, Hm, Wm, Ha, Wa, int(size[0]), int(size[1])))


def label_epilogue_hist(main, aux, size, hist, num_classes, lut=None, want_kld=False):
    main = _f32(main, 'main')
    N, C, Hm, Wm = main.shape
    Ha = Wa = 0
    if aux is not None:
        aux = _f32(aux, 'aux')
        if aux.shape[0] != N or aux.shape[1] != C:
            raise RuntimeError('mspl_amd: aux logits %s do not match main %s' % (tuple(aux.shape), tuple(main.shape)))
        Ha, Wa = aux.shape[2:]
    H, W = int(size[0]), int(size[1])
    if hist.dtype != torch.int64 or not hist.is_cuda or hist.numel() < num_classes:
        raise RuntimeError('mspl_amd: hist must be a CUDA int64 tensor with >= num_classes entries')
    if lut is not None and (lut.dtype != torch.uint8 or not lut.is_cuda or lut.numel() < C):
        raise RuntimeError('mspl_amd: lut must be a CUDA uint8 tensor with >= %d entries' % C)
    res = {'labels': torch.empty((N, H, W), device=main.device, dtype=torch.uint8)}
    if want_kld:
        res['kld'] = torch.empty((N, H, W), device=main.device, dtype=torch.float32)
    nbytes = int(lib.mspl_label_epilogue_hist_workspace_bytes(N, H, W))
    ws = torch.empty(max(nbytes, 4), device=main.device, dtype=torch.uint8)
    check(lib.mspl_label_epilogue_hist_fwd(_p(main), _p(aux), N, C, Hm, Wm, Ha, Wa, H, W, _p(lut), _p(res['labels']),
                                           _p(res.get('kld')), _p(hist), int(num_classes), _p(ws), nbytes, _stream()))
    return res


def merge_labels(sources, num_classes, thresh, fill=4, hist=None):
    S = len(sources)
    if S < 1:
        raise RuntimeError('mspl_amd: merge_labels needs at least one source')
    src = []
    for t in sources:
        if t.dtype != torch.uint8 or not t.is_cuda:
            raise RuntimeError('mspl_amd: merge_labels sources must be CUDA uint8 tensors')
        if t.shape != sources[0].shape:
            raise RuntimeError('mspl_amd: merge_labels sources differ in shape')
        src.append(t.contiguous())
    out = torch.empty_like(src[0])
    if hist is not None and (hist.dtype != torch.int64 or not hist.is_cuda or hist.numel() < num_classes):
        raise RuntimeError('mspl_amd: hist must be a CUDA int64 tensor with >= num_classes entries')
    arr = (ctypes.c_void_p * S)(*[t.data_ptr() for t in src])
    check(lib.mspl_merge_labels_fwd(arr, S, out.numel(), num_classes, int(thresh), int(fill), _p(out), _p(hist),
                                    _stream()))
    return out
```

### mspl_amd/uest.py

```python
import numpy as np
import torch

from . import layers, ops

id_camvid_to_greenhouse = np.array([4, 2, 2, 3, 3, 1, 2, 2, 2, 4, 4, 2, 4])
id_cityscapes_to_greenhouse = np.array([3, 3, 2, 2, 2, 2, 2, 2, 1, 3, 4, 4, 4, 2, 2, 2, 2, 2, 2, 4])
id_forest_to_greenhouse = np.array([3, 1, 1, 2, 2])
LUTS = {'camvid': id_camvid_to_greenhouse, 'cityscapes': id_cityscapes_to_greenhouse,
        'forest': id_forest_to_greenhouse}
GREENHOUSE_CLASSES = 5
NO_AGREEMENT_CLASS = 4


def resolve_thresh(num_data, thresh):
    if thresh is None or thresh == 'half':
        return num_data // 2 + 1
    if thresh == 'all':
        return num_data
    if isinstance(thresh, int) and not isinstance(thresh, bool) and thresh <= num_data:
        return thresh
    return num_data // 2 + 1


def _lowres(model, image, pyr=None):
    out = model.forward_lowres(image, pyr=pyr) if pyr is not None else model.forward_lowres(image)
    return out if isinstance(out, tuple) else (out, None)


def _lowres_batch_stats(model, images, pyr=None):
    mains, auxs = [], []
    for k in range(images.shape[0]):
        with torch.enable_grad():
            main, aux = _lowres(model, images[k:k + 1], pyr)
        mains.append(main.detach())
        auxs.append(None if aux is None else aux.detach())
    return torch.cat(mains), (None if auxs[0] is None else torch.cat(auxs))


def get_output(model, image, model_name='espdnetue', device='cuda'):
    with torch.no_grad():
        image = image.to(device)
        main, aux = _lowres(model, image)
        r = ops.label_epilogue(main, aux, image.shape[2:], want_labels=False, want_prob=True, want_kld=True)
    return r['prob'][0].cpu().numpy(), r['kld'][0].cpu().numpy()


def merge_outputs(amax_outputs, seg_classes=GREENHOUSE_CLASSES, thresh=None):
    is_np = isinstance(amax_outputs, np.ndarray)
    t = torch.from_numpy(np.ascontiguousarray(amax_outputs).astype(np.uint8)).cuda() if is_np else amax_outputs
    if t.dtype != torch.uint8:
        t = t.to(torch.uint8)
    S = t.shape[0]
    if t[0].numel() == 0:
        out = torch.empty_like(t[0])
    else:
        out = ops.merge_labels([t[s] for s in range(S)], seg_classes, resolve_thresh(S, thresh), NO_AGREEMENT_CLASS)
    return out.cpu().numpy().astype(np.int64) if is_np else out


def class_weights_from_histogram(class_array, policy='normal'):
    class_array = np.asarray(class_array, dtype=np.float64)
    if policy == 'normal':
        freq = class_array / class_array.sum()
        w = 1.0 / (freq + 1e-10)
        w[0] = 0.0
        return w
    return np.ones(len(class_array))


import os as _os
_NO_SIGNATURE = _os.environ.get('MSPL_GRAPH_SIGNATURE', '1') == '0'


class _GraphedPassMixin:

    def _signature(self):
        if _NO_SIGNATURE:
            return (layers._PARAM_EPOCH[0],)
        slots = self.__dict__.get('_sig_slots')
        if slots is None:
            slots = []
            for m in self._graph_models():
                for mod in m.modules():
                    slots += [(mod._parameters, k) for k, t in mod._parameters.items() if t is not None and t.is_floating_point()]
                    slots += [(mod._buffers, k) for k, t in mod._buffers.items() if t is not None and t.is_floating_point()]
            self._sig_slots = slots
        sig = [layers._PARAM_EPOCH[0]]
        for d, k in slots:
            t = d.get(k)
            sig.append(None if t is None else (id(t), t.data_ptr(), t._version))
        return tuple(sig)

    def invalidate_graphs(self):
        self._graphs.clear()
        self.__dict__.pop('_sig_slots', None)

    def _cache_tensors(self):
        keep = []
        for m in self._graph_models():
            for mod in m.modules():
                for _, val in mod.__dict__.get('_mspl_cache', {}).values():
                    keep.append(val)
        return keep

    def _replay(self, images, copy_always=False):
        key = self._shape_key(images)
        sig = self._signature()
        g = self._graphs.get(key)
        if g is not None and g.signature != sig:
# ... 12 lines not shown
                t.copy_(b)
            graph = torch.cuda.CUDAGraph()
            with torch.cuda.graph(graph, capture_error_mode='thread_local'):
                static_out = self._graph_outputs(self._run(static_in))
            for t, b in zip(state, before):
                t.copy_(b)
            graph._mspl_keep = (static_in, state, self._cache_tensors(), list(getattr(self, 'luts', ())))
            g = self._graphs[key] = _Captured(graph, static_in, static_out, sig)
        self._copy_input(g.static_in, images, copy_always)
        g.graph.replay()
        return g.static_out

    @staticmethod
    def _shape_key(images):
        return tuple(images.shape)

    def _graph_state(self):
        return [self.hist]

    @staticmethod
    def _clone_input(images):
        return images.clone()

    @staticmethod
    def _copy_input(static_in, images, copy_always):
        if copy_always or static_in.data_ptr() != images.data_ptr():
            static_in.copy_(images)

    def static_input(self, shape):
        g = self._graphs.get(tuple(shape))
        if g is None:
            return None
        view = g.static_in.view(g.static_in.shape)
        view._mspl_graph = g.graph
        return view


class _Captured(object):
    __slots__ = ('graph', 'static_in', 'static_out', 'signature')

    def __init__(self, graph, static_in, static_out, signature):
        self.graph, self.static_in, self.static_out, self.signature = graph, static_in, static_out, signature

    def __iter__(self):
        return iter((self.graph, self.static_in, self.static_out))

    def __getitem__(self, i):
        return (self.graph, self.static_in, self.static_out)[i]


class PseudoLabelPass(_GraphedPassMixin):

    def __init__(self, model_list, os_data_list, classes=GREENHOUSE_CLASSES, merge_label_policy='all',
                 device='cuda', use_graph=False, eval_training=False):
        if len(model_list) != len(os_data_list) or not model_list:
            raise ValueError('model_list and os_data_list must be non-empty and of equal length')
        self.eval_training = bool(eval_training)
        self.models = [(m.to(device).train() if self.eval_training else m.to(device).eval()) for m in model_list]
        self.os_data = list(os_data_list)
        self.classes = classes
        self.thresh = resolve_thresh(len(model_list), merge_label_policy)
        self.device = torch.device(device)
        self.luts = []
        for m, d in zip(self.models, self.os_data):
            lut = LUTS.get(d)
            self.luts.append(None if lut is None else torch.from_numpy(lut.astype(np.uint8)).to(self.device))
        self.hist = torch.zeros(classes, dtype=torch.int64, device=self.device)
        self.use_graph = use_graph and not self.eval_training
        self._graphs = {}

    def reset(self):
        self.hist.zero_()

    def _run(self, images):
        maps = []
        if self.eval_training:
            for m, lut in zip(self.models, self.luts):
                main, aux = _lowres_batch_stats(m, images)
                maps.append(ops.label_epilogue(main, aux, images.shape[2:], lut=lut)['labels'])
            return ops.merge_labels(maps, self.classes, self.thresh, NO_AGREEMENT_CLASS, self.hist), maps
        shared = all(hasattr(m, 'depth_base_net') and getattr(m.base_net, 'input_reinforcement', False) for m in self.models)
        pyr = layers.ImagePyramid(images) if shared and len(self.models) > 1 else None
        for m, lut in zip(self.models, self.luts):
            main, aux = _lowres(m, images, pyr)
            maps.append(ops.label_epilogue(main, aux, images.shape[2:], lut=lut)['labels'])
        return ops.merge_labels(maps, self.classes, self.thresh, NO_AGREEMENT_CLASS, self.hist), maps

    def source_maps(self, images):
        with torch.no_grad():
            return self._run(images.to(self.device))[1]

    def __call__(self, images):
        with torch.no_grad():
            images = images.to(self.device)
            if not self.use_graph:
                return self._run(images)[0]
            return self._replay(images)

    def _graph_models(self):
        return self.models

    @staticmethod
    def _graph_outputs(run_result):
        return run_result[0]

    def class_weights(self, policy='normal'):
        return torch.from_numpy(class_weights_from_histogram(self.hist.cpu().numpy(), policy)).float().to(self.device)


def _concurrent_streams(n, device, candidates=12, spin_cycles=400000):
    import time
    if n == 1 or not hasattr(torch.cuda, '_sleep'):
        return [torch.cuda.Stream(device=device) for _ in range(n)]

    def spin_ms(streams):
        torch.cuda.synchronize(device)
        t0 = time.perf_counter()
        for st in streams:
            with torch.cuda.stream(st):
                torch.cuda._sleep(spin_cycles)
        torch.cuda.synchronize(device)
        return (time.perf_counter() - t0) * 1e3

    pool = [torch.cuda.Stream(device=device) for _ in range(candidates)]
    for _ in range(30):
        spin_ms(pool[:1])
    chosen = [pool[0]]
    for attempt in range(3):
        one = min(spin_ms(pool[:1]) for _ in range(3))
        chosen = [pool[0]]
        for st in pool[1:]:
            if len(chosen) == n:
                break
            if min(spin_ms(chosen + [st]) for _ in range(2)) < one * (1.0 + 0.5 * len(chosen)):
                chosen.append(st)
        if len(chosen) < n:
            break
        together = min(spin_ms(chosen) for _ in range(3))
        alone = min(spin_ms(chosen[:1]) for _ in range(3))
        if together < 1.6 * alone:
            break
    while len(chosen) < n:
        chosen.append(torch.cuda.Stream(device=device))
    return chosen


class PipelinedLabelPass:

    def __init__(self, make_pass, depth=3, device='cuda', group=1):
        if depth < 1 or group < 1:
            raise ValueError('PipelinedLabelPass: depth and group must be >= 1')
        self.device = torch.device(device)
        self.depth, self.group = depth, group
        self.lanes = [make_pass() for _ in range(depth)]
        self.streams = _concurrent_streams(depth, self.device)
        self._pending = []
        self._n = 0
        self._staged = None
        self._lane_no = 0
        self._bufs = {}

    def join(self):
        cur = torch.cuda.current_stream(self.device)
        for st in self.streams:
            cur.wait_stream(st)

# ... 144 lines not shown
    for b, batch in enumerate(testloader):
        if world > 1 and not pre_sharded and b % world != rank:
            continue
        image = batch[0]
        names.append(list(batch[-2]))
        batch_sizes.append(len(names[-1]))
        if transform is not None:
            slot = None
            if hasattr(p, 'static_inputs'):
                W, H = transform.size
                shape = (image.shape[0], 3, H, W)
                xs = slots.get(shape)
                if not xs or any(x is None for x in xs):
                    xs = slots[shape] = p.static_inputs(shape)
                slot = xs[p.next_lane] if xs else None
            if on_lane:
                with torch.cuda.stream(p.next_stream):
                    image = transform(image, out=slot)
            else:
                image = transform(image, out=slot)
            image = image[0] if isinstance(image, tuple) else image
        elif not (image.is_cuda or eager_input):
            image = image.to(device, non_blocking=True)
        out = p(image, on_lane=True) if on_lane else p(image)
        if out is not None:
            consume(out)
    for out in (p.flush(on_lane=True) if on_lane else p.flush()):
        consume(out)
    lists = writer.close()
    hist = p.hist
    if mdist.collective_needed():
        recs, at = [], 0
        for n in batch_sizes:
            recs.append(tuple(l[at:at + n] for l in lists))
            at += n
        merged_recs = mdist.gather_lists(recs)
        lists = tuple([x for r in merged_recs for x in r[k]] for k in range(len(lists)))
        hist = mdist.reduce_histogram(hist.clone())
    if rank == 0:
        update_image_list(tgt_train_lst, *lists)
    mdist.barrier()
    weights = torch.from_numpy(class_weights_from_histogram(hist.cpu().numpy(), class_weighting)).float().to(hist.device)
    return tgt_train_lst, weights


def generate_pseudo_label_multi_model(model_list, os_data_list, testloader, save_path, classes=GREENHOUSE_CLASSES,
                                      merge_label_policy='all', class_weighting='normal', use_depth=False, device='cuda',
                                      use_graph=True, writer_workers=None, in_flight=3, pre_sharded=False, _label_pass=None,
                                      batches_per_launch=1, transform=None, eval_training=False):
    p = _label_pass if _label_pass is not None else PipelinedLabelPass(
        lambda: PseudoLabelPass(model_list, os_data_list, classes=classes, merge_label_policy=merge_label_policy,
                                device=device, use_graph=use_graph, eval_training=eval_training),
        depth=1 if eval_training else in_flight, device=device, group=1 if eval_training else batches_per_launch)
    return _label_loop(p, testloader, save_path, lambda out: out, class_weighting, use_depth, device, writer_workers, pre_sharded,
                       transform, _label_pass is not None)


def generate_pseudo_label(model, testloader, save_path, classes=GREENHOUSE_CLASSES, class_weighting='normal', use_depth=False,
                          device='cuda', use_graph=True, writer_workers=None, in_flight=3, batches_per_launch=2, pre_sharded=False,
                          _label_pass=None, transform=None, eval_training=False):
    p = _label_pass if _label_pass is not None else PipelinedLabelPass(
        lambda: SelfLabelPass(model, classes=classes, device=device, use_graph=use_graph, with_kld=False, eval_training=eval_training),
        depth=1 if eval_training else in_flight, device=device, group=1 if eval_training else batches_per_launch)
    return _label_loop(p, testloader, save_path, lambda out: out[0] if isinstance(out, (tuple, list)) else out, class_weighting,
                       use_depth, device, writer_workers, pre_sharded, transform, _label_pass is not None)


class SelfLabelPass(_GraphedPassMixin):

    def __init__(self, model, classes=GREENHOUSE_CLASSES, device='cuda', use_graph=False, with_kld=True, eval_training=False):
        self.eval_training = bool(eval_training)
        self.model = model.to(device).train() if self.eval_training else model.to(device).eval()
        self.classes = classes
        self.device = torch.device(device)
        self.hist = torch.zeros(classes, dtype=torch.int64, device=self.device)
        self.use_graph = use_graph and not self.eval_training
        self.with_kld = with_kld
        self._graphs = {}

    def reset(self):
        self.hist.zero_()

    def _run(self, images):
        main, aux = _lowres_batch_stats(self.model, images) if self.eval_training else _lowres(self.model, images)
        if main.shape[1] <= min(24, self.classes, 32) and ops.label_epilogue_hist_fits(main, aux, images.shape[2:]):
            r = ops.label_epilogue_hist(main, aux, images.shape[2:], self.hist, self.classes, want_kld=self.with_kld)
            return r['labels'], r.get('kld')
        r = ops.label_epilogue(main, aux, images.shape[2:], want_kld=self.with_kld)
        labels = ops.merge_labels([r['labels']], self.classes, 1, NO_AGREEMENT_CLASS, self.hist)
        return labels, r.get('kld')

    def __call__(self, images):
        with torch.no_grad():
            images = images.to(self.device)
            if not self.use_graph:
                return self._run(images)
            return self._replay(images)

    def _graph_models(self):
        return [self.model]

    @staticmethod
    def _graph_outputs(run_result):
        return run_result
```

Before: 21570 images/s.

## Fuse final 1x1 classifier heads into the label epilogue kernel

Adds a label epilogue kernel that takes the decoder's 16-plane feature maps plus the head weights and biases, computes the 1x1 classifier logits for the main and aux heads on the fly in shared memory, then does bilinear upsampling, argmax, KL and histogram in the same pass. The model gets a forward_heads path that stops before the final 1x1 convs. This removes the separate head conv launches and the write and re-read of the low-res logit tensors. In exchange the tile staging reads 16 feature planes instead of 13 logit planes, and the path only activates when shape and thin-conv predicates hold. The shared pixel and setup code is factored into include files.

```diff
diff --git a/include/mspl_hip.h b/include/mspl_hip.h
--- a/include/mspl_hip.h
+++ b/include/mspl_hip.h
@@ -152,6 +152,16 @@
                                  int32_t Hm, int32_t Wm, int32_t Ha, int32_t Wa, int32_t H, int32_t W,
                                  const uint8_t* lut, uint8_t* labels, float* kld, unsigned long long* hist,
                                  int32_t num_classes, void* workspace, int64_t workspace_bytes, void* stream);
+
+int mspl_label_epilogue_heads_fits(int32_t N, int32_t C, int32_t P, int32_t Hm, int32_t Wm, int32_t Ha, int32_t Wa,
+                                   int32_t H, int32_t W);
+int mspl_label_epilogue_heads_fwd(const float* main_feat, const float* main_w, const float* main_b,
+                                  const float* aux_feat, const float* aux_w, const float* aux_b, int32_t N, int32_t C,
+                                  int32_t P, int32_t Hm, int32_t Wm, int32_t Ha, int32_t Wa, int32_t H, int32_t W,
+                                  const uint8_t* lut, uint8_t* labels, float* kld, unsigned long long* hist,
+                                  int32_t num_classes, void* workspace, int64_t workspace_bytes, void* stream);
+
+int mspl_conv1x1_chain_order(int32_t N, int32_t Cin, int32_t Cout, int32_t groups, int32_t HW);
 
 int mspl_merge_labels_fwd(const uint8_t* const* src, int32_t S, int64_t npix, int32_t num_classes,
                           int32_t thresh, int32_t fill, uint8_t* out, unsigned long long* hist,
diff --git a/mspl_amd/_native.py b/mspl_amd/_native.py
--- a/mspl_amd/_native.py
+++ b/mspl_amd/_native.py
@@ -84,6 +84,10 @@
                                      ctypes.c_void_p],
     'mspl_label_epilogue_hist_workspace_bytes': [c_i32, c_i32, c_i32],
     'mspl_label_epilogue_hist_fits': [c_i32] * 8,
+    'mspl_label_epilogue_heads_fits': [c_i32] * 9,
+    'mspl_conv1x1_chain_order': [c_i32] * 5,
+    'mspl_label_epilogue_heads_fwd': [c_f32p] * 6 + [c_i32] * 9 + [ctypes.c_void_p, ctypes.c_void_p, c_f32p, ctypes.c_void_p, c_i32,
+                                                                   ctypes.c_void_p, c_i64, ctypes.c_void_p],
     'mspl_conv_bwd_data': [c_f32p, c_f32p] + [c_i32] * 10 + [c_f32p, ctypes.c_void_p],
     'mspl_conv_bwd_weight': [c_f32p, c_f32p] + [c_i32] * 10 + [c_f32p, ctypes.c_void_p],
     'mspl_affine_prelu_bwd': [c_f32p] * 7 + [c_i32] * 3 + [c_f32p] * 5 + [ctypes.c_void_p],
diff --git a/mspl_amd/csrc/conv1x1.hip b/mspl_amd/csrc/conv1x1.hip
--- a/mspl_amd/csrc/conv1x1.hip
+++ b/mspl_amd/csrc/conv1x1.hip
@@ -755,13 +755,19 @@
     }
 }
 
-static int launch_thin_try(const float* x, const float* w, int N, int Cin, int Cout, int groups, int HW, const Epi& e, float* out,
-                           hipStream_t s) {
+static bool thin_shape(int N, int Cin, int Cout, int groups, int HW) {
     static const int enabled = MSPL_TUNE_INT("MSPL_PW_THIN", 1);
     const int K = Cin / groups, M = Cout / groups;
     if (!enabled || M > 16 || K < 8 || K > 64 || (K & 7) != 0 || (HW & 3) != 0 ||
         (int64_t)N * groups * ceil_div(HW / 4, 256) < 400)
-        return 1;
+        return false;
+    return (size_t)groups * K * (M <= 8 ? 8 : 16) * sizeof(float) <= 48 * 1024 && (int64_t)N * groups < 65535ll * 65535ll;
+}
+
+static int launch_thin_try(const float* x, const float* w, int N, int Cin, int Cout, int groups, int HW, const Epi& e, float* out,
+                           hipStream_t s) {
+    const int K = Cin / groups, M = Cout / groups;
+    if (!thin_shape(N, Cin, Cout, groups, HW)) return 1;
     if (((uintptr_t)x & 15) || ((uintptr_t)out & 15) || ((uintptr_t)e.raw & 15) || ((uintptr_t)e.pre_add & 15) ||
         ((uintptr_t)e.residual & 15) || ((uintptr_t)e.reinf_r & 15) || ((uintptr_t)e.gate & 15))
         return 1;
@@ -930,6 +936,11 @@
     else hipLaunchKernelGGL(conv1x1_valu_kernel<8>, grid, blk, lds, s, x, w, g, e, out);
     MSPL_CHECK_LAUNCH("conv1x1(small-K)");
     return MSPL_OK;
+}
+
+extern "C" int mspl_conv1x1_chain_order(int32_t N, int32_t Cin, int32_t Cout, int32_t groups, int32_t HW) {
+    if (N <= 0 || Cin <= 0 || Cout <= 0 || groups <= 0 || HW <= 0 || Cin % groups || Cout % groups) return 0;
+    return thin_shape(N, Cin, Cout, groups, HW) ? 1 : 0;
 }
 
 extern "C" int mspl_conv1x1_fwd(const float* x, const float* w, int32_t N, int32_t Cin, int32_t Cout,
diff --git a/mspl_amd/csrc/label_epilogue_pixels.inc b/mspl_amd/csrc/label_epilogue_pixels.inc
--- /dev/null
+++ b/mspl_amd/csrc/label_epilogue_pixels.inc
@@ -0,0 +1,136 @@
+    __syncthreads();
+
+    const int wms_c = WMS > 0 ? WMS : st.wms, was_c = WAS > 0 ? WAS : st.was;
+    const int x = xb + tid;
+    unsigned int cnt_mask_lo = 0;
+    if (x < g.W) {
+#pragma clang fp contract(fast)
+        int mx0, mx1, ax0 = 0, ax1 = 0;  float mwx0, mwx1, awx0 = 0.f, awx1 = 0.f;
+        bilinear_src(g.swm, x, g.Wm, mx0, mx1, mwx0, mwx1);
+        if (auxp) bilinear_src(g.swa, x, g.Wa, ax0, ax1, awx0, awx1);
+        const float* mcol = ml + (mx0 - cmA);
+        const float* acol = al + (ax0 - caA);
+        const int mdx = mx1 - mx0, adx = ax1 - ax0;
+        float mtop[CMAX], mbot[CMAX], atop[CMAX], abot[CMAX];
+        int mkt = -1, mkb = -1, akt = -1, akb = -1;
+#pragma unroll
+        for (int c = 0; c < CMAX; ++c) { mtop[c] = mbot[c] = atop[c] = abot[c] = 0.f; }
+#pragma unroll 1
+        for (int r = 0; r < LE_RB; ++r) {
+            const int y = y0 + r;
+            unsigned lab8 = 0xffu;
+            if (y < g.H) {
+                int my0, my1;  float mwy0, mwy1;
+                bilinear_src(g.shm, y, g.Hm, my0, my1, mwy0, mwy1);
+                if (my0 != mkt) {
+                    if (my0 == mkb) {
+#pragma unroll
+                        for (int c = 0; c < CMAX; ++c) mtop[c] = mbot[c];
+                    } else {
+                        const float* mr0 = mcol + (my0 - rm_lo) * (EXACT ? CMAX : g.C) * wms_c;
+                        const float* mr0b = mr0 + mdx;
+#pragma unroll
+                        for (int c = 0; c < CMAX; ++c)
+                            if (EXACT || c < g.C) mtop[c] = mwx0 * mr0[c * wms_c] + mwx1 * mr0b[c * wms_c];
+                    }
+                    mkt = my0;
+                }
+                if (my1 != mkb) {
+                    if (my1 == mkt) {
+#pragma unroll
+                        for (int c = 0; c < CMAX; ++c) mbot[c] = mtop[c];
+                    } else {
+                        const float* mr1 = mcol + (my1 - rm_lo) * (EXACT ? CMAX : g.C) * wms_c;
+                        const float* mr1b = mr1 + mdx;
+#pragma unroll
+                        for (int c = 0; c < CMAX; ++c)
+                            if (EXACT || c < g.C) mbot[c] = mwx0 * mr1[c * wms_c] + mwx1 * mr1b[c * wms_c];
+                    }
+                    mkb = my1;
+                }
+                float m[CMAX], a[CMAX];
+#pragma unroll
+                for (int c = 0; c < CMAX; ++c) m[c] = (EXACT || c < g.C) ? mwy0 * mtop[c] + mwy1 * mbot[c] : -INFINITY;
+                if (auxp) {
+                    int ay0, ay1;  float awy0, awy1;
+                    bilinear_src(g.sha, y, g.Ha, ay0, ay1, awy0, awy1);
+                    if (ay0 != akt) {
+                        if (ay0 == akb) {
+#pragma unroll
+                            for (int c = 0; c < CMAX; ++c) atop[c] = abot[c];
+                        } else {
+                            const float* ar0 = acol + (ay0 - ra_lo) * (EXACT ? CMAX : g.C) * was_c;
+                            const float* ar0b = ar0 + adx;
+#pragma unroll
+                            for (int c = 0; c < CMAX; ++c)
+                                if (EXACT || c < g.C) atop[c] = awx0 * ar0[c * was_c] + awx1 * ar0b[c * was_c];
+                        }
+                        akt = ay0;
+                    }
+                    if (ay1 != akb) {
+                        if (ay1 == akt) {
+#pragma unroll
+                            for (int c = 0; c < CMAX; ++c) abot[c] = atop[c];
+                        } else {
+                            const float* ar1 = acol + (ay1 - ra_lo) * (EXACT ? CMAX : g.C) * was_c;
+                            const float* ar1b = ar1 + adx;
+#pragma unroll
+                            for (int c = 0; c < CMAX; ++c)
+                                if (EXACT || c < g.C) abot[c] = awx0 * ar1[c * was_c] + awx1 * ar1b[c * was_c];
+                        }
+                        akb = ay1;
+                    }
+#pragma unroll
+                    for (int c = 0; c < CMAX; ++c) a[c] = (EXACT || c < g.C) ? awy0 * atop[c] + awy1 * abot[c] : -INFINITY;
+                } else {
+#pragma unroll
+                    for (int c = 0; c < CMAX; ++c) a[c] = (EXACT || c < g.C) ? 0.f : -INFINITY;
+                }
+                const size_t pix = ((size_t)n * g.H + y) * g.W + x;
+                if (labels) {
+                    float omax = -INFINITY;  int best = 0;
+#pragma unroll
+                    for (int c = 0; c < CMAX; ++c) {
+                        if (EXACT || c < g.C) { const float o = m[c] + 0.5f * a[c]; if (o > omax) { omax = o; best = c; } }
+                    }
+                    lab8 = lut ? (unsigned)lut[best] : (unsigned)best;
+                    labels[pix] = (uint8_t)lab8;
+                }
+                if (kld) {
+                    float k = 0.f;
+                    if (auxp) {
+                        float M1 = -INFINITY, M2 = -INFINITY;
+#pragma unroll
+                        for (int c = 0; c < CMAX; ++c) { M1 = fmaxf(M1, m[c]); M2 = fmaxf(M2, a[c]); }
+                        float S1 = 0.f, T1 = 0.f, S2 = 0.f;
+#pragma unroll
+                        for (int c = 0; c < CMAX; ++c) {
+                            if (EXACT || c < g.C) {
+                                const float d1 = m[c] - M1, d2 = a[c] - M2;
+                                const float e1 = __expf(d1);
+                                S1 += e1;
+                                T1 = fmaf(e1, d1 - d2, T1);
+                                S2 += __expf(d2);
+                            }
+                        }
+                        k = T1 / S1 - __logf(S1) + __logf(S2);
+                    }
+                    kld[pix] = k;
+                }
+            }
+            cnt_mask_lo |= lab8 << (8 * r);
+        }
+    } else {
+        cnt_mask_lo = 0xffffffffu;
+    }
+    if (hist_ws) {
+        for (int c = 0; c < st.ncls; ++c) {
+            unsigned cnt = 0;
+#pragma unroll
+            for (int r = 0; r < LE_RB; ++r)
+                cnt += (unsigned)__builtin_popcountll(__builtin_amdgcn_ballot_w64(((cnt_mask_lo >> (8 * r)) & 0xffu) == (unsigned)c));
+            if ((tid & 63) == 0 && cnt) atomicAdd(&sh_hist[c], cnt);
+        }
+        __syncthreads();
+        if (tid < 32) hist_ws[(size_t)blk * 32 + tid] = tid < st.ncls ? sh_hist[tid] : 0u;
+    }
diff --git a/mspl_amd/csrc/label_epilogue_setup.inc b/mspl_amd/csrc/label_epilogue_setup.inc
--- /dev/null
+++ b/mspl_amd/csrc/label_epilogue_setup.inc
@@ -0,0 +1,29 @@
+    extern __shared__ __attribute__((aligned(16))) float smem[];
+    float* ml = smem;
+    float* al = smem + (size_t)st.nrm * g.C * st.wms;
+    unsigned int* sh_hist = reinterpret_cast<unsigned int*>(al + (size_t)st.nra * g.C * st.was);
+    const int tid = threadIdx.x;
+    const int xb = blockIdx.x * 256;
+    const int nbands = (g.H + LE_RB - 1) / LE_RB;
+    const int bq = (nbands + 3) >> 2;
+    const int band = (int)(blockIdx.y & 3) * bq + (int)(blockIdx.y >> 2), n = blockIdx.z;
+    const unsigned blk = (blockIdx.z * gridDim.y + blockIdx.y) * gridDim.x + blockIdx.x;
+    if (band >= nbands) {
+        if (hist_ws && tid < 32) hist_ws[(size_t)blk * 32 + tid] = 0u;
+        return;
+    }
+    const int y0 = band * LE_RB;
+    const int ylast = min(y0 + LE_RB, g.H) - 1, xlast = min(xb + 256, g.W) - 1;
+    int rm_lo, rm_hi, cm_lo, cm_hi, t0, t1;  float f0, f1;
+    bilinear_src(g.shm, y0, g.Hm, rm_lo, t1, f0, f1);
+    bilinear_src(g.shm, ylast, g.Hm, t0, rm_hi, f0, f1);
+    bilinear_src(g.swm, xb, g.Wm, cm_lo, t1, f0, f1);
+    bilinear_src(g.swm, xlast, g.Wm, t0, cm_hi, f0, f1);
+    int ra_lo = 0, ra_hi = -1, ca_lo = 0, ca_hi = -1;
+    if (auxp) {
+        bilinear_src(g.sha, y0, g.Ha, ra_lo, t1, f0, f1);
+        bilinear_src(g.sha, ylast, g.Ha, t0, ra_hi, f0, f1);
+        bilinear_src(g.swa, xb, g.Wa, ca_lo, t1, f0, f1);
+        bilinear_src(g.swa, xlast, g.Wa, t0, ca_hi, f0, f1);
+    }
+    if (hist_ws && tid < 32) sh_hist[tid] = 0;
diff --git a/mspl_amd/csrc/labels.hip b/mspl_amd/csrc/labels.hip
--- a/mspl_amd/csrc/labels.hip
+++ b/mspl_amd/csrc/labels.hip
@@ -187,36 +187,7 @@
                                                                  LeGeom g, LeStage st, const uint8_t* __restrict__ lut,
                                                                  uint8_t* __restrict__ labels, float* __restrict__ kld,
                                                                  unsigned int* __restrict__ hist_ws) {
-    extern __shared__ __attribute__((aligned(16))) float smem[];
-    float* ml = smem;
-    float* al = smem + (size_t)st.nrm * g.C * st.wms;
-    unsigned int* sh_hist = reinterpret_cast<unsigned int*>(al + (size_t)st.nra * g.C * st.was);
-    const int tid = threadIdx.x;
-    const int xb = blockIdx.x * 256;
-    const int nbands = (g.H + LE_RB - 1) / LE_RB;
-    const int bq = (nbands + 3) >> 2;
-    const int band = (int)(blockIdx.y & 3) * bq + (int)(blockIdx.y >> 2), n = blockIdx.z;
-    const unsigned blk = (blockIdx.z * gridDim.y + blockIdx.y) * gridDim.x + blockIdx.x;
-    if (band >= nbands) {
-        if (hist_ws && tid < 32) hist_ws[(size_t)blk * 32 + tid] = 0u;
-        return;
-    }
-    const int y0 = band * LE_RB;
-    const int ylast = min(y0 + LE_RB, g.H) - 1, xlast = min(xb + 256, g.W) - 1;
-    int rm_lo, rm_hi, cm_lo, cm_hi, t0, t1;  float f0, f1;
-    bilinear_src(g.shm, y0, g.Hm, rm_lo, t1, f0, f1);
-    bilinear_src(g.shm, ylast, g.Hm, t0, rm_hi, f0, f1);
-    bilinear_src(g.swm, xb, g.Wm, cm_lo, t1, f0, f1);
-    bilinear_src(g.swm, xlast, g.Wm, t0, cm_hi, f0, f1);
-    int ra_lo = 0, ra_hi = -1, ca_lo = 0, ca_hi = -1;
-    if (auxp) {
-        bilinear_src(g.sha, y0, g.Ha, ra_lo, t1, f0, f1);
-        bilinear_src(g.sha, ylast, g.Ha, t0, ra_hi, f0, f1);
-        bilinear_src(g.swa, xb, g.Wa, ca_lo, t1, f0, f1);
-        bilinear_src(g.swa, xlast, g.Wa, t0, ca_hi, f0, f1);
-    }
-    if (hist_ws && tid < 32) sh_hist[tid] = 0;
-
+#include "label_epilogue_setup.inc"
     const int cmA = st.vec ? (cm_lo & ~3) : cm_lo, caA = st.vec ? (ca_lo & ~3) : ca_lo;
     {
         const int mplane = g.Hm * g.Wm, aplane = g.Ha * g.Wa;
@@ -290,142 +261,122 @@
             }
         }
     }
+#include "label_epilogue_pixels.inc"
+}
+
+constexpr int LE_HP = 16;
+
+struct LeHeads {
+    const float* wm;  const float* bm;
+    const float* wa;  const float* ba;
+};
+
+template <int CMAX, int WMS, int WAS>
+__global__ __launch_bounds__(256) void label_epilogue_heads_kernel(
+        const float* __restrict__ mainp, const float* __restrict__ auxp, LeGeom g, LeStage st, LeHeads hd,
+        const uint8_t* __restrict__ lut, uint8_t* __restrict__ labels, float* __restrict__ kld, unsigned int* __restrict__ hist_ws) {
+    constexpr bool EXACT = true;
+#include "label_epilogue_setup.inc"
+    const int cmA = cm_lo & ~3, caA = ca_lo & ~3;
+    {
+    constexpr int G = (CMAX + 3) / 4, CP = 4 * G;
+    float* wl = reinterpret_cast<float*>(sh_hist + 32);
+    float* bl = wl + 2 * LE_HP * CP;
+    for (int i = tid; i < 2 * LE_HP * CP; i += 256) {
+        const int c = i % CP, k = (i / CP) % LE_HP;
+        const float* w = i < LE_HP * CP ? hd.wm : hd.wa;
+        wl[i] = (c < CMAX && w) ? w[c * LE_HP + k] : 0.f;
+    }
+    for (int i = tid; i < 2 * CP; i += 256) {
+        const int c = i % CP;
+        const float* b = i < CP ? hd.bm : hd.ba;
+        bl[i] = (c < CMAX && b) ? b[c] : 0.f;
+    }
     __syncthreads();
-
-    const int wms_c = WMS > 0 ? WMS : st.wms, was_c = WAS > 0 ? WAS : st.was;
-    const int x = xb + tid;
-    unsigned int cnt_mask_lo = 0;
-    if (x < g.W) {
-#pragma clang fp contract(fast)
-        int mx0, mx1, ax0 = 0, ax1 = 0;  float mwx0, mwx1, awx0 = 0.f, awx1 = 0.f;
-        bilinear_src(g.swm, x, g.Wm, mx0, mx1, mwx0, mwx1);
-        if (auxp) bilinear_src(g.swa, x, g.Wa, ax0, ax1, awx0, awx1);
-        const float* mcol = ml + (mx0 - cmA);
-        const float* acol = al + (ax0 - caA);
-        const int mdx = mx1 - mx0, adx = ax1 - ax0;
-        float mtop[CMAX], mbot[CMAX], atop[CMAX], abot[CMAX];
-        int mkt = -1, mkb = -1, akt = -1, akb = -1;
-#pragma unroll
-        for (int c = 0; c < CMAX; ++c) { mtop[c] = mbot[c] = atop[c] = abot[c] = 0.f; }
+    constexpr int UNR = CMAX <= 8 ? 4 : 8;
+    const int mplane = g.Hm * g.Wm, aplane = g.Ha * g.Wa;
+    const float* mb = mainp + (size_t)n * LE_HP * mplane;
+    const float* ab = auxp ? auxp + (size_t)n * LE_HP * aplane : nullptr;
+    const int cqm = st.wms >> 2, cqa = st.was >> 2;
+    const int ntm = (rm_hi - rm_lo + 1) * cqm, nta = (auxp && hd.wa) ? (ra_hi - ra_lo + 1) * cqa : 0;
+    const int wms_s = WMS > 0 ? WMS : st.wms, was_s = WAS > 0 ? WAS : st.was;
+    for (int t = tid; t < ntm + nta; t += 256) {
+        const bool ism = t < ntm;
+        const int tt = ism ? t : t - ntm, cq = ism ? cqm : cqa;
+        const int row = (int)((unsigned)tt / (unsigned)cq), q = tt - row * cq;
+        const int col = (ism ? cmA : caA) + 4 * q;
+        if (!(col < (ism ? g.Wm : g.Wa) && col <= (ism ? cm_hi : ca_hi))) continue;
+        const int plane = ism ? mplane : aplane;
+        const float* src = ism ? mb + (rm_lo + row) * g.Wm + col : ab + (ra_lo + row) * g.Wa + col;
+        const float* wt = wl + (ism ? 0 : LE_HP * CP);
+        float acc[CMAX][4];
+#pragma unroll
+        for (int c = 0; c < CMAX; ++c) acc[c][0] = acc[c][1] = acc[c][2] = acc[c][3] = 0.f;
 #pragma unroll 1
-        for (int r = 0; r < LE_RB; ++r) {
-            const int y = y0 + r;
-            unsigned lab8 = 0xffu;
-            if (y < g.H) {
-                int my0, my1;  float mwy0, mwy1;
-                bilinear_src(g.shm, y, g.Hm, my0, my1, mwy0, mwy1);
-                if (my0 != mkt) {
-                    if (my0 == mkb) {
-#pragma unroll
-                        for (int c = 0; c < CMAX; ++c) mtop[c] = mbot[c];
-                    } else {
-                        const float* mr0 = mcol + (my0 - rm_lo) * (EXACT ? CMAX : g.C) * wms_c;
-                        const float* mr0b = mr0 + mdx;
-#pragma unroll
-                        for (int c = 0; c < CMAX; ++c)
-                            if (EXACT || c < g.C) mtop[c] = mwx0 * mr0[c * wms_c] + mwx1 * mr0b[c * wms_c];
+        for (int k0 = 0; k0 < LE_HP; k0 += UNR) {
+            float4 xv[UNR];
+#pragma unroll
+            for (int u = 0; u < UNR; ++u) xv[u] = *reinterpret_cast<const float4*>(src + (size_t)(k0 + u) * plane);
+            __builtin_amdgcn_sched_barrier(0);
+#pragma unroll
+            for (int u = 0; u < UNR; ++u) {
+#pragma unroll
+                for (int c4 = 0; c4 < CP; c4 += 4) {
+                    const float4 wv = *reinterpret_cast<const float4*>(wt + (k0 + u) * CP + c4);
+                    const float ww[4] = {wv.x, wv.y, wv.z, wv.w};
+#pragma unroll
+                    for (int i = 0; i < 4; ++i) {
+                        if (c4 + i < CMAX) {
+                            acc[c4 + i][0] = fmaf(ww[i], xv[u].x, acc[c4 + i][0]);
+                            acc[c4 + i][1] = fmaf(ww[i], xv[u].y, acc[c4 + i][1]);
+                            acc[c4 + i][2] = fmaf(ww[i], xv[u].z, acc[c4 + i][2]);
+                            acc[c4 + i][3] = fmaf(ww[i], xv[u].w, acc[c4 + i][3]);
+                        }
                     }
-                    mkt = my0;
                 }
-                if (my1 != mkb) {
-                    if (my1 == mkt) {
-#pragma unroll
-                        for (int c = 0; c < CMAX; ++c) mbot[c] = mtop[c];
-                    } else {
-                        const float* mr1 = mcol + (my1 - rm_lo) * (EXACT ? CMAX : g.C) * wms_c;
-                        const float* mr1b = mr1 + mdx;
-#pragma unroll
-                        for (int c = 0; c < CMAX; ++c)
-                            if (EXACT || c < g.C) mbot[c] = mwx0 * mr1[c * wms_c] + mwx1 * mr1b[c * wms_c];
-                    }
-                    mkb = my1;
+            }
+        }
+        const int cst = ism ? wms_s : was_s;
+        float* dst = (ism ? ml : al) + row * CMAX * cst + 4 * q;
+        const float* bt = bl + (ism ? 0 : CP);
+#pragma unroll
+        for (int c = 0; c < CMAX; ++c) {
+            const float b = bt[c];
+            *reinterpret_cast<float4*>(dst + c * cst) =
+                make_float4(fmaf(acc[c][0], 1.0f, b), fmaf(acc[c][1], 1.0f, b), fmaf(acc[c][2], 1.0f, b), fmaf(acc[c][3], 1.0f, b));
+        }
+    }
+    if (auxp && !hd.wa) {
+        const int wavei = __builtin_amdgcn_readfirstlane(tid >> 6), lane = tid & 63;
+        const float* lb = auxp + (size_t)n * CMAX * aplane;
+        const int npair = (ra_hi - ra_lo + 1) * CMAX;
+        const int ppw = cqa <= 64 ? 64 / cqa : 1;
+        const int slot = (int)(((unsigned)lane * st.magqa) >> 20), q = lane - slot * cqa;
+        const int col = caA + 4 * q;
+        const bool lane_ok = slot < ppw && col < g.Wa && col <= ca_hi;
+        const float* base = lb + (size_t)ra_lo * g.Wa + col;
+        float* dbase = al + 4 * q;
+        constexpr int UL = 4;
+        for (int p0 = wavei * ppw + slot; p0 - slot < npair; p0 += 4 * ppw * UL) {
+            float4 v[UL];  int dst[UL];
+#pragma unroll
+            for (int u = 0; u < UL; ++u) {
+                const int pair = p0 + u * 4 * ppw;
+                dst[u] = -1;  v[u] = make_float4(0.f, 0.f, 0.f, 0.f);
+                if (lane_ok && pair < npair) {
+                    const int row = (int)(((unsigned)pair * st.magc) >> 16), cc = pair - row * CMAX;
+                    v[u] = *reinterpret_cast<const float4*>(base + (size_t)cc * aplane + row * g.Wa);
+                    dst[u] = pair * was_s;
                 }
-                float m[CMAX], a[CMAX];
-#pragma unroll
-                for (int c = 0; c < CMAX; ++c) m[c] = (EXACT || c < g.C) ? mwy0 * mtop[c] + mwy1 * mbot[c] : -INFINITY;
-                if (auxp) {
-                    int ay0, ay1;  float awy0, awy1;
-                    bilinear_src(g.sha, y, g.Ha, ay0, ay1, awy0, awy1);
-                    if (ay0 != akt) {
-                        if (ay0 == akb) {
-#pragma unroll
-                            for (int c = 0; c < CMAX; ++c) atop[c] = abot[c];
-                        } else {
-                            const float* ar0 = acol + (ay0 - ra_lo) * (EXACT ? CMAX : g.C) * was_c;
-                            const float* ar0b = ar0 + adx;
-#pragma unroll
-                            for (int c = 0; c < CMAX; ++c)
-                                if (EXACT || c < g.C) atop[c] = awx0 * ar0[c * was_c] + awx1 * ar0b[c * was_c];
-                        }
-                        akt = ay0;
-                    }
-                    if (ay1 != akb) {
-                        if (ay1 == akt) {
-#pragma unroll
-                            for (int c = 0; c < CMAX; ++c) abot[c] = atop[c];
-                        } else {
-                            const float* ar1 = acol + (ay1 - ra_lo) * (EXACT ? CMAX : g.C) * was_c;
-                            const float* ar1b = ar1 + adx;
-#pragma unroll
-                            for (int c = 0; c < CMAX; ++c)
-                                if (EXACT || c < g.C) abot[c] = awx0 * ar1[c * was_c] + awx1 * ar1b[c * was_c];
-                        }
-                        akb = ay1;
-                    }
-#pragma unroll
-                    for (int c = 0; c < CMAX; ++c) a[c] = (EXACT || c < g.C) ? awy0 * atop[c] + awy1 * abot[c] : -INFINITY;
-                } else {
-#pragma unroll
-                    for (int c = 0; c < CMAX; ++c) a[c] = (EXACT || c < g.C) ? 0.f : -INFINITY;
-                }
-                const size_t pix = ((size_t)n * g.H + y) * g.W + x;
-                if (labels) {
-                    float omax = -INFINITY;  int best = 0;
-#pragma unroll
-                    for (int c = 0; c < CMAX; ++c) {
-                        if (EXACT || c < g.C) { const float o = m[c] + 0.5f * a[c]; if (o > omax) { omax = o; best = c; } }
-                    }
-                    lab8 = lut ? (unsigned)lut[best] : (unsigned)best;
-                    labels[pix] = (uint8_t)lab8;
-                }
-                if (kld) {
-                    float k = 0.f;
-                    if (auxp) {
-                        float M1 = -INFINITY, M2 = -INFINITY;
-#pragma unroll
-                        for (int c = 0; c < CMAX; ++c) { M1 = fmaxf(M1, m[c]); M2 = fmaxf(M2, a[c]); }
-                        float S1 = 0.f, T1 = 0.f, S2 = 0.f;
-#pragma unroll
-                        for (int c = 0; c < CMAX; ++c) {
-                            if (EXACT || c < g.C) {
-                                const float d1 = m[c] - M1, d2 = a[c] - M2;
-                                const float e1 = __expf(d1);
-                                S1 += e1;
-                                T1 = fmaf(e1, d1 - d2, T1);
-                                S2 += __expf(d2);
-                            }
-                        }
-                        k = T1 / S1 - __logf(S1) + __logf(S2);
-                    }
-                    kld[pix] = k;
-                }
-            }
-            cnt_mask_lo |= lab8 << (8 * r);
-        }
-    } else {
-        cnt_mask_lo = 0xffffffffu;
-    }
-    if (hist_ws) {
-        for (int c = 0; c < st.ncls; ++c) {
-            unsigned cnt = 0;
-#pragma unroll
-            for (int r = 0; r < LE_RB; ++r)
-                cnt += (unsigned)__builtin_popcountll(__builtin_amdgcn_ballot_w64(((cnt_mask_lo >> (8 * r)) & 0xffu) == (unsigned)c));
-            if ((tid & 63) == 0 && cnt) atomicAdd(&sh_hist[c], cnt);
-        }
-        __syncthreads();
-        if (tid < 32) hist_ws[(size_t)blk * 32 + tid] = tid < st.ncls ? sh_hist[tid] : 0u;
-    }
+            }
+            __builtin_amdgcn_sched_barrier(0);
+#pragma unroll
+            for (int u = 0; u < UL; ++u)
+                if (dst[u] >= 0) *reinterpret_cast<float4*>(dbase + dst[u]) = v[u];
+        }
+    }
+    }
+#include "label_epilogue_pixels.inc"
 }
 
 constexpr int LE_RED = 16;
@@ -713,6 +664,104 @@
                                workspace, workspace_bytes, stream);
 }
 
+struct LeHeadsPlan {
+    LeGeom g;
+    LeStage st;
+    size_t lds;
+    bool wide480;
+};
+
+static bool le_heads_plan(int N, int C, int P, int Hm, int Wm, int Ha, int Wa, int H, int W, LeHeadsPlan& pl) {
+    if (N <= 0 || Hm <= 0 || Wm <= 0 || H <= 0 || W <= 0 || Ha < 0 || Wa < 0 || (Ha > 0) != (Wa > 0)) return false;
+    if (P != LE_HP || !(C == 5 || C == 13 || C == 20)) return false;
+    const bool aux = Ha > 0;
+    if ((Wm & 3) || (aux && (Wa & 3))) return false;
+    const int cmax = std::max(C, P);
+    if (!(H <= 65535 * LE_RB / 4 && N <= 65535 && (int64_t)N * cmax * Hm * Wm < (1ll << 31) &&
+          (int64_t)N * cmax * (int64_t)Ha * Wa < (1ll << 31) && (int64_t)N * H * W < (1ll << 31)))
+        return false;
+    LeGeom& g = pl.g;
+    g.N = N; g.C = C; g.Hm = Hm; g.Wm = Wm; g.Ha = Ha; g.Wa = Wa; g.H = H; g.W = W;
+    g.shm = bilinear_scale(Hm, H); g.swm = bilinear_scale(Wm, W);
+    g.sha = aux ? bilinear_scale(Ha, H) : 0.f; g.swa = aux ? bilinear_scale(Wa, W) : 0.f;
+    LeStage& st = pl.st;
+    st.vec = 1;
+    st.nrm = bilinear_span(Hm, H, LE_RB, false);  st.wms = bilinear_span(Wm, W, 256, true);
+    st.nra = aux ? bilinear_span(Ha, H, LE_RB, false) : 0;  st.was = aux ? bilinear_span(Wa, W, 256, true) : 4;
+    st.ncls = 0;
+    st.magc = (65536u + (unsigned)C - 1) / (unsigned)C;
+    st.magqm = 0;
+    st.magqa = ((1u << 20) + (unsigned)(st.was >> 2) - 1) / (unsigned)(st.was >> 2);
+    for (int k = 0; k < 64; ++k)
+        if ((int)(((unsigned)k * st.magqa) >> 20) != k / (st.was >> 2)) return false;
+    if (st.nra * C >= 4096) return false;
+    const int G = (C + 3) / 4;
+    pl.lds = ((size_t)st.nrm * C * st.wms + (size_t)st.nra * C * st.was + 32 + 2 * (size_t)(4 * G) * (LE_HP + 1)) * sizeof(float);
+    pl.wide480 = st.wms == 132 && (!aux || st.was == 68);
+    return pl.lds <= 128 * 1024 && st.wms <= 256 && st.was <= 256;
+}
+
+extern "C" int mspl_label_epilogue_heads_fits(int32_t N, int32_t C, int32_t P, int32_t Hm, int32_t Wm, int32_t Ha, int32_t Wa,
+                                              int32_t H, int32_t W) {
+    LeHeadsPlan pl;
+    return le_heads_plan(N, C, P, Hm, Wm, Ha, Wa, H, W, pl) ? 1 : 0;
+}
+
+extern "C" int mspl_label_epilogue_heads_fwd(const float* main_feat, const float* main_w, const float* main_b,
+                                             const float* aux_feat, const float* aux_w, const float* aux_b, int32_t N, int32_t C,
+                                             int32_t P, int32_t Hm, int32_t Wm, int32_t Ha, int32_t Wa, int32_t H, int32_t W,
+                                             const uint8_t* lut, uint8_t* labels, float* kld, unsigned long long* hist,
+                                             int32_t num_classes, void* workspace, int64_t workspace_bytes, void* stream) {
+    MSPL_REQUIRE(main_feat && main_w, MSPL_ERR_NULL_POINTER, "label_epilogue_heads: null main features or weight");
+    MSPL_REQUIRE(labels || kld, MSPL_ERR_NULL_POINTER, "label_epilogue_heads: no output requested");
+    MSPL_REQUIRE(!hist || labels, MSPL_ERR_NULL_POINTER, "label_epilogue_heads: the histogram counts the labels written");
+    MSPL_REQUIRE(!hist || (num_classes >= 1 && num_classes <= 32), MSPL_ERR_UNSUPPORTED, "label_epilogue_heads: %d classes (1..32)",
+                 num_classes);
+    if (!aux_feat) Ha = Wa = 0;
+    LeHeadsPlan pl;
+    MSPL_REQUIRE(le_heads_plan(N, C, P, Hm, Wm, Ha, Wa, H, W, pl), MSPL_ERR_UNSUPPORTED,
+                 "label_epilogue_heads: shape outside the heads form (N=%d C=%d P=%d main=%dx%d aux=%dx%d out=%dx%d); "
+                 "ask mspl_label_epilogue_heads_fits", N, C, P, Hm, Wm, Ha, Wa, H, W);
+    MSPL_REQUIRE(((((uintptr_t)main_feat) | ((uintptr_t)aux_feat)) & 15) == 0, MSPL_ERR_UNSUPPORTED,
+                 "label_epilogue_heads: feature maps must be 16-byte aligned");
+    hipStream_t st_ = (hipStream_t)stream;
+    unsigned int* ws = nullptr;
+    if (hist) {
+        const int64_t need = le_blocks(N, H, W) * 32 * (int64_t)sizeof(unsigned int);
+        MSPL_REQUIRE(workspace && workspace_bytes >= need, MSPL_ERR_BAD_SHAPE,
+                     "label_epilogue_heads: workspace of %lld bytes, need %lld (mspl_label_epilogue_hist_workspace_bytes)",
+                     (long long)workspace_bytes, (long long)need);
+        ws = (unsigned int*)workspace;
+        pl.st.ncls = num_classes;
+    }
+    static const bool big_lds = [] {
+        bool ok = true;
+#define MSPL_LEH_ATTR(CM, A, B) ok = hipFuncSetAttribute((const void*)label_epilogue_heads_kernel<CM, A, B>, hipFuncAttributeMaxDynamicSharedMemorySize, 128 * 1024) == hipSuccess && ok
+        MSPL_LEH_ATTR(5, 0, 0);  MSPL_LEH_ATTR(5, 132, 68);
+        MSPL_LEH_ATTR(13, 0, 0); MSPL_LEH_ATTR(13, 132, 68);
+        MSPL_LEH_ATTR(20, 0, 0); MSPL_LEH_ATTR(20, 132, 68);
+#undef MSPL_LEH_ATTR
+        (void)hipGetLastError();
+        return ok;
+    }();
+    MSPL_REQUIRE(big_lds || pl.lds <= 64 * 1024, MSPL_ERR_HIP, "label_epilogue_heads: could not raise the dynamic LDS limit");
+    LeHeads hd;
+    hd.wm = main_w; hd.bm = main_b; hd.wa = aux_feat ? aux_w : nullptr; hd.ba = (aux_feat && aux_w) ? aux_b : nullptr;
+    const dim3 grid((unsigned)ceil_div(W, 256), (unsigned)(4 * ceil_div(ceil_div(H, LE_RB), 4)), (unsigned)N);
+#define MSPL_LEH_LAUNCH(CM) do { if (pl.wide480) hipLaunchKernelGGL((label_epilogue_heads_kernel<CM, 132, 68>), grid, dim3(256), pl.lds, st_, main_feat, aux_feat, pl.g, pl.st, hd, lut, labels, kld, ws); \
+                                 else hipLaunchKernelGGL((label_epilogue_heads_kernel<CM, 0, 0>), grid, dim3(256), pl.lds, st_, main_feat, aux_feat, pl.g, pl.st, hd, lut, labels, kld, ws); } while (0)
+    if (C == 5) MSPL_LEH_LAUNCH(5);
+    else if (C == 13) MSPL_LEH_LAUNCH(13);
+    else MSPL_LEH_LAUNCH(20);
+#undef MSPL_LEH_LAUNCH
+    MSPL_CHECK_LAUNCH("label_epilogue_heads");
+    if (hist) {
+        hipLaunchKernelGGL(label_hist_reduce_kernel, dim3(LE_RED), dim3(256), 0, st_, ws, (int)le_blocks(N, H, W), num_classes, hist);
+        MSPL_CHECK_LAUNCH("label_epilogue_heads(histogram)");
+    }
+    return MSPL_OK;
+}
+
 extern "C" int mspl_merge_labels_fwd(const uint8_t* const* src, int32_t S, int64_t npix, int32_t num_classes,
                                      int32_t thresh, int32_t fill, uint8_t* out, unsigned long long* hist,
                                      void* stream) {
diff --git a/mspl_amd/layers.py b/mspl_amd/layers.py
--- a/mspl_amd/layers.py
+++ b/mspl_amd/layers.py
@@ -68,6 +68,28 @@
     def __exit__(self, *exc):
         global _SIDE_ENABLED
         _SIDE_ENABLED = self.prev
+
+
+_LABEL_HEADS = False
+
+
+class label_heads(object):
+
+    def __init__(self, enabled):
+        self.enabled = enabled
+
+    def __enter__(self):
+        global _LABEL_HEADS
+        self.prev = _LABEL_HEADS
+        _LABEL_HEADS = bool(self.enabled)
+
+    def __exit__(self, *exc):
+        global _LABEL_HEADS
+        _LABEL_HEADS = self.prev
+
+
+def label_heads_enabled():
+    return _LABEL_HEADS
 
 
 def _side_stream(idx, device, parent):
@@ -704,7 +726,7 @@
             return ag.conv_affine_prelu(out, conv.weight, 1, 1, None, conv.bias, None)
         return ag.affine_prelu(ag.conv(out, conv.weight, 1, 1), None, conv.bias, None)
 
-    def forward(self, x, fused=True, projected=False):
+    def forward(self, x, fused=True, projected=False, heads=False):
         if _training_path():
             return self._forward_train(x)
         if not projected:
@@ -714,6 +736,8 @@
         ok = fused and self._fusable(sizes, height, width) and all(
             (s >= 1.0) or (hs <= height and ws <= width) for s, (hs, ws) in zip(self.scales, sizes))
         m = self.forward_fused(x, sizes) if ok else self.forward_unfused(x)
+        if heads and not self.last_layer_br:
+            return m, self.merge_layer[3].weight, self.merge_layer[3].bias
         return ops.conv1x1(m, self.merge_layer[3].weight, 1, self._final_epilogue())
 
 
diff --git a/mspl_amd/models.py b/mspl_amd/models.py
--- a/mspl_amd/models.py
+++ b/mspl_amd/models.py
@@ -186,7 +186,7 @@
             l4 = self.fusion_gate_level4(l4, dl4)
         return l1, l2, l3, l4
 
-    def _decode(self, l1, l2, l3, l4, aux_layer):
+    def _decode(self, l1, l2, l3, l4, aux_layer, heads=False, aux_heads=True):
         aux = None
         st2 = (self.merge_enc_dec_l2, self.bu_br_l2, self.bu_dec_l2)
         st3 = (self.merge_enc_dec_l3, self.bu_br_l3, self.bu_dec_l3)
@@ -207,31 +207,31 @@
         bu = self.bu_dec_l1(l4)
         if aux_layer == 0:
             with fork(2, (bu,)):
-                aux = self.aux_decoder(bu)
+                aux = self.aux_decoder(bu, heads=heads and aux_heads)
         wait_mark(e2, (pw2,))
         bu = self._decode_stage(st2, l3, pw2, bu)
         if aux_layer == 1:
             with fork(2, (bu,)):
-                aux = self.aux_decoder(bu)
+                aux = self.aux_decoder(bu, heads=heads and aux_heads)
         wait_mark(e3, (pw3,))
         bu = self._decode_stage(st3, l2, pw3, bu)
         if aux_layer == 2:
             with fork(2, (bu,)):
-                aux = self.aux_decoder(bu)
+                aux = self.aux_decoder(bu, heads=heads and aux_heads)
         wait_mark(e4, (pw4,))
-        bu = self._decode_stage(st4, l1, pw4, bu)
-        join(2, (aux,))
+        bu = self._decode_stage(st4, l1, pw4, bu, heads)
+        join(2, (aux[0] if isinstance(aux, tuple) else aux,))
         return bu, aux
 
     @staticmethod
-    def _decode_stage(st, enc, pw, bu):
+    def _decode_stage(st, enc, pw, bu, heads=False):
         merge, br, pyr = st
         if pw.dim() == 2:
             proj = decoder_stage_fused(merge, enc, pw, bu, br, pyr)
             if proj is not None:
-                return pyr(proj, projected=True)
+                return pyr(proj, projected=True, heads=heads)
             pw = merge.expand(enc, pw)
-        return pyr(decoder_merge(pw, bu, br))
+        return pyr(decoder_merge(pw, bu, br), heads=heads)
 
     def get_basenet_params(self):
         return _param_gen([self.base_net])
@@ -286,6 +286,15 @@
         l1, l2, l3, l4 = self._encode_rgbd(x, x_d)
         return self._decode(l1, l2, l3, l4, self.aux_layer)
 
+    def forward_heads(self, x, x_d=None, pyr=None, aux_features=True):
+        _check_input(x)
+        if x_d is None:
+            l1, l2, l3, l4 = self._encode(x, True, self.depth_base_net.level3, pyr)
+        else:
+            l1, l2, l3, l4 = self._encode_rgbd(x, x_d)
+        main, aux = self._decode(l1, l2, l3, l4, self.aux_layer, heads=True, aux_heads=aux_features)
+        return main, (aux if aux is None or isinstance(aux, tuple) else (aux, None, None))
+
     def forward(self, x, x_d=None):
         main, aux = self.forward_lowres(x, x_d)
         if _training_path():
@@ -325,6 +334,14 @@
             l1, l2, l3, l4 = self._encode_rgbd(x, x_d)
         return self._decode(l1, l2, l3, l4, -1)[0], None
 
+    def forward_heads(self, x, x_d=None, pyr=None):
+        _check_input(x)
+        if x_d is None:
+            l1, l2, l3, l4 = self._encode(x, True, self.depth_base_net.level3, pyr)
+        else:
+            l1, l2, l3, l4 = self._encode_rgbd(x, x_d)
+        return self._decode(l1, l2, l3, l4, -1, heads=True)[0], None
+
     def forward(self, x, x_d=None):
         main, _ = self.forward_lowres(x, x_d)
         if _training_path():
@@ -345,6 +362,13 @@
         _check_input(x)
         l1, l2, l3, l4 = self._encode(x, False, self.base_net.level3)
         return self._decode(l1, l2, l3, l4, -1)[0], None
+
+    def forward_heads(self, x, x_d=None, pyr=None):
+        if x_d is not None:
+            raise RuntimeError('mspl_amd: ESPNetv2Segmentation has no depth branch')
+        _check_input(x)
+        l1, l2, l3, l4 = self._encode(x, False, self.base_net.level3, pyr)
+        return self._decode(l1, l2, l3, l4, -1, heads=True)[0], None
 
     def forward(self, x):
         main, _ = self.forward_lowres(x)
diff --git a/mspl_amd/ops.py b/mspl_amd/ops.py
--- a/mspl_amd/ops.py
+++ b/mspl_amd/ops.py
@@ -619,6 +619,74 @@
     return res
 
 
+def head_logits(head):
+    m, w, b = head
+    return conv1x1(m, w, 1, Epi(shift=b))
+
+
+def conv1x1_chain_order(x_shape, cout, groups=1):
+    N, Cin, H, W = [int(v) for v in x_shape]
+    return bool(lib.mspl_conv1x1_chain_order(N, Cin, int(cout), int(groups), H * W))
+
+
+def _head_args(head, name):
+    m, w, b = head
+    if w is None:
+        return _f32(m, name + ' logits'), None, None
+    m, w = _f32(m, name + ' features'), _f32(w, name + ' weight')
+    C, P = int(w.shape[0]), int(m.shape[1])
+    if w.numel() != C * P:
+        raise RuntimeError('mspl_amd: %s weight %s does not match %d feature planes' % (name, tuple(w.shape), P))
+    return m, w, _vec(b, C, name + ' bias')
+
+
+def label_epilogue_heads_fits(main, aux, size):
+    N, P, Hm, Wm = [int(v) for v in main[0].shape]
+    C = int(main[1].shape[0])
+    Ha = Wa = 0
+    if aux is not None:
+        if int(aux[0].shape[0]) != N or (int(aux[0].shape[1]) != C if aux[1] is None else
+                                         (int(aux[0].shape[1]) != P or int(aux[1].shape[0]) != C)):
+            return False
+        Ha, Wa = [int(v) for v in aux[0].shape[2:]]
+    return label_epilogue_heads_fits_shape(N, C, P, Hm, Wm, Ha, Wa, int(size[0]), int(size[1]))
+
+
+def label_epilogue_heads_fits_shape(N, C, P, Hm, Wm, Ha, Wa, H, W):
+    return bool(lib.mspl_label_epilogue_heads_fits(int(N), int(C), int(P), int(Hm), int(Wm), int(Ha), int(Wa), int(H), int(W)))
+
+
+def label_epilogue_heads(main, aux, size, hist=None, num_classes=0, lut=None, want_labels=True, want_kld=False):
+    m, wm, bm = _head_args(main, 'main')
+    N, P, Hm, Wm = m.shape
+    C = int(wm.shape[0])
+    a = wa = ba = None
+    Ha = Wa = 0
+    if aux is not None:
+        a, wa, ba = _head_args(aux, 'aux')
+        if a.shape[0] != N or (a.shape[1] != C if wa is None else (a.shape[1] != P or wa.shape[0] != C)):
+            raise RuntimeError('mspl_amd: aux head %s does not match main %s x %s' % (tuple(a.shape), tuple(m.shape), tuple(wm.shape)))
+        Ha, Wa = a.shape[2:]
+    H, W = int(size[0]), int(size[1])
+    if lut is not None and (lut.dtype != torch.uint8 or not lut.is_cuda or lut.numel() < C):
+        raise RuntimeError('mspl_amd: lut must be a CUDA uint8 tensor with >= %d entries' % C)
+    res = {}
+    if want_labels:
+        res['labels'] = torch.empty((N, H, W), device=m.device, dtype=torch.uint8)
+    if want_kld:
+        res['kld'] = torch.empty((N, H, W), device=m.device, dtype=torch.float32)
+    ws, nbytes = None, 0
+    if hist is not None:
+        if hist.dtype != torch.int64 or not hist.is_cuda or hist.numel() < num_classes:
+            raise RuntimeError('mspl_amd: hist must be a CUDA int64 tensor with >= num_classes entries')
+        nbytes = int(lib.mspl_label_epilogue_hist_workspace_bytes(N, H, W))
+        ws = torch.empty(max(nbytes, 4), device=m.device, dtype=torch.uint8)
+    check(lib.mspl_label_epilogue_heads_fwd(_p(m), _p(wm), _p(bm), _p(a), _p(wa), _p(ba), N, C, P, Hm, Wm, Ha, Wa, H, W, _p(lut),
+                                            _p(res.get('labels')), _p(res.get('kld')), _p(hist), int(num_classes), _p(ws), nbytes,
+                                            _stream()))
+    return res
+
+
 def merge_labels(sources, num_classes, thresh, fill=4, hist=None):
     S = len(sources)
     if S < 1:
diff --git a/mspl_amd/uest.py b/mspl_amd/uest.py
--- a/mspl_amd/uest.py
+++ b/mspl_amd/uest.py
@@ -25,6 +25,27 @@
 def _lowres(model, image, pyr=None):
     out = model.forward_lowres(image, pyr=pyr) if pyr is not None else model.forward_lowres(image)
     return out if isinstance(out, tuple) else (out, None)
+
+
+def _heads(model, image, pyr=None):
+    fh = getattr(model, 'forward_heads', None)
+    dec = getattr(model, 'bu_dec_l4', None)
+    if fh is None or dec is None or not layers.label_heads_enabled() or image.shape[2] % 16 or image.shape[3] % 16:
+        return None
+    N, _, H, W = [int(v) for v in image.shape]
+    conv = dec.merge_layer[3]
+    C, P = conv.out_channels, conv.in_channels
+    al = getattr(model, 'aux_layer', -1) if hasattr(model, 'aux_decoder') else -1
+    Ha, Wa = ((H >> (4 - al), W >> (4 - al)) if 0 <= al < 3 else (0, 0))
+    if dec.last_layer_br or not ops.label_epilogue_heads_fits_shape(N, C, P, H // 2, W // 2, Ha, Wa, H, W) \
+            or not ops.conv1x1_chain_order((N, P, H // 2, W // 2), C):
+        return None
+    aux_features = Ha > 0 and ops.conv1x1_chain_order((N, P, Ha, Wa), C)
+    kw = {} if pyr is None else {'pyr': pyr}
+    main, aux = fh(image, aux_features=aux_features, **kw) if Ha > 0 else fh(image, **kw)
+    if not ops.label_epilogue_heads_fits(main, aux, image.shape[2:]):
+        raise RuntimeError('mspl_amd: the heads of %s are not the shapes predicted from the input %s' % (type(model).__name__, tuple(image.shape)))
+    return main, aux
 
 
 def _lowres_batch_stats(model, images, pyr=None):
@@ -203,6 +224,10 @@
         shared = all(hasattr(m, 'depth_base_net') and getattr(m.base_net, 'input_reinforcement', False) for m in self.models)
         pyr = layers.ImagePyramid(images) if shared and len(self.models) > 1 else None
         for m, lut in zip(self.models, self.luts):
+            hd = _heads(m, images, pyr)
+            if hd is not None:
+                maps.append(ops.label_epilogue_heads(hd[0], hd[1], images.shape[2:], lut=lut)['labels'])
+                continue
             main, aux = _lowres(m, images, pyr)
             maps.append(ops.label_epilogue(main, aux, images.shape[2:], lut=lut)['labels'])
         return ops.merge_labels(maps, self.classes, self.thresh, NO_AGREEMENT_CLASS, self.hist), maps
@@ -513,6 +538,10 @@
         self.hist.zero_()
 
     def _run(self, images):
+        hd = None if self.eval_training or getattr(self.model, 'classes', 1 << 30) > min(24, self.classes, 32) else _heads(self.model, images)
+        if hd is not None:
+            r = ops.label_epilogue_heads(hd[0], hd[1], images.shape[2:], self.hist, self.classes, want_kld=self.with_kld)
+            return r['labels'], r.get('kld')
         main, aux = _lowres_batch_stats(self.model, images) if self.eval_training else _lowres(self.model, images)
         if main.shape[1] <= min(24, self.classes, 32) and ops.label_epilogue_hist_fits(main, aux, images.shape[2:]):
             r = ops.label_epilogue_hist(main, aux, images.shape[2:], self.hist, self.classes, want_kld=self.with_kld)
```

Result: no change. 21500 images/s (-0.4%).
